# genome-vendor/allpathslg

Hardware: NVIDIA B200
Metric: k-mer spectrum throughput (K=25), k-mer instances counted per second (higher is better)
Workload: dtype u64

## Files before the change

allpathslg_b200/_lib.py:

```python
import ctypes as C
import os

_HERE = os.path.dirname(os.path.abspath(__file__))
LIB_PATH = os.path.join(_HERE, "libapgk.so")

APGK_OK = 0
E_ARG, E_CUDA, E_NOMEM, E_STATE, E_RANGE = -1, -2, -3, -4, -5
WANT_SPECTRUM, WANT_COUNTS, ASYNC_INGEST = 1, 2, 4
N_STAGES = 14
MAX_K = 96


class Config(C.Structure):
    _fields_ = [("K", C.c_int32), ("device", C.c_int32), ("flags", C.c_uint32), ("prefix_bits", C.c_int32),
                ("reserve_bases", C.c_uint64), ("max_round_keys", C.c_uint64),
                ("max_inner_keys", C.c_uint64)]


class GroupStats(C.Structure):
    _fields_ = [("world", C.c_int32), ("n_rounds", C.c_int32), ("n_outer_rounds", C.c_int32), ("prefix_bits", C.c_int32),
                ("split_bits", C.c_int32), ("peer_exchange", C.c_int32), ("shard_instances", C.c_uint64),
                ("remote_bytes", C.c_uint64), ("gather_ms", C.c_float), ("step_ms", C.c_float)]


class GroupFreqStats(C.Structure):
    _fields_ = [("n_batches", C.c_int32), ("n_queries", C.c_uint64), ("remote_bytes", C.c_uint64), ("sweep_ms", C.c_float),
                ("exchange_ms", C.c_float), ("scatter_ms", C.c_float), ("total_ms", C.c_float)]


class SynthParams(C.Structure):
    _fields_ = [("genome_len", C.c_uint64), ("seed_g", C.c_uint64), ("seed_p", C.c_uint64), ("seed_q", C.c_uint64),
                ("seed_r", C.c_uint64), ("seed_e", C.c_uint64), ("read_len", C.c_uint32), ("err_per_200", C.c_uint32)]


_u64p = C.POINTER(C.c_uint64)
_u32p = C.POINTER(C.c_uint32)
_vp = C.c_void_p
SYMBOLS = {
    "apgk_create": (C.c_int, [C.POINTER(Config), C.POINTER(_vp)]),
    "apgk_destroy": (None, [_vp]),
    "apgk_last_error": (C.c_char_p, [_vp]),
    "apgk_words_per_kmer": (C.c_int, [C.c_int]),
    "apgk_reset": (C.c_int, [_vp]),
    "apgk_add_reads": (C.c_int, [_vp, _vp, _vp, C.c_uint64]),
    "apgk_add_reads_uniform": (C.c_int, [_vp, _vp, C.c_uint64, C.c_uint64, C.c_uint32]),
    "apgk_synth_reads": (C.c_int, [_vp, C.POINTER(SynthParams), C.c_uint64, C.c_uint64]),
    "apgk_export_reads": (C.c_int, [_vp, _vp]),
    "apgk_read_store_info": (C.c_int, [_vp, _u64p, _u64p]),
    "apgk_finish": (C.c_int, [_vp]),
    "apgk_totals": (C.c_int, [_vp, _u64p, _u64p]),
    "apgk_spectrum": (C.c_int, [_vp, C.POINTER(_u64p), _u64p]),
    "apgk_spectrum_sparse": (C.c_int, [_vp, C.POINTER(_u64p), C.POINTER(_u64p), _u64p]),
    "apgk_counts_device": (C.c_int, [_vp, C.POINTER(_vp), C.POINTER(_vp), _u64p]),
    "apgk_counts_copy": (C.c_int, [_vp, C.c_uint64, C.c_uint64, _vp, _vp]),
    "apgk_reserve_table": (C.c_int, [_vp, C.c_uint64]),
    "apgk_release_temp": (C.c_int, [_vp]),
    "apgk_prefix_range": (C.c_int, [_vp, C.c_int32, C.c_uint64, _u64p, _u64p]),
    "apgk_lookup": (C.c_int, [_vp, _vp, C.c_uint64, C.c_int, _vp]),
    "apgk_read_freqs": (C.c_int, [_vp, C.c_uint64, C.c_uint64, _vp]),
    "apgk_read_freqs_device": (C.c_int, [_vp, _vp, C.POINTER(C.c_float)]),
    "apgk_build_occurrences": (C.c_int, [_vp]),
    "apgk_occurrences_info": (C.c_int, [_vp, _u64p, _u64p, C.POINTER(C.c_float)]),
    "apgk_occurrences_device": (C.c_int, [_vp, C.POINTER(_vp), C.POINTER(_vp), _u64p]),
    "apgk_occurrences_copy": (C.c_int, [_vp, C.c_uint64, C.c_uint64, _vp, _vp, _vp]),
    "apgk_owner_plan": (C.c_int, [_vp, C.c_uint32, _vp]),
    "apgk_owner_scatter": (C.c_int, [_vp, _vp]),
    "apgk_key_buffer": (C.c_int, [_vp, C.c_uint64, C.POINTER(_vp)]),
    "apgk_owner_of": (C.c_int, [C.c_int, _vp, C.c_uint64, C.c_uint32, _vp]),
    "apgk_finish_keys_device": (C.c_int, [_vp, _vp, C.c_uint64]),
    "apgk_window_upper": (C.c_int, [_vp, C.POINTER(C.c_uint64)]),
    "apgk_choose_prefix_bits": (C.c_int, [_vp, C.c_uint64, C.POINTER(C.c_int32)]),
    "apgk_partition": (C.c_int, [_vp, C.c_int32]),
    "apgk_partition_range": (C.c_int, [_vp, C.c_int32, C.c_int32, C.c_int32]),
    "apgk_level0_totals": (C.c_int, [_vp, _vp, C.c_uint32, C.POINTER(C.c_uint32), C.POINTER(C.c_uint64)]),
    "apgk_partition_info": (C.c_int, [_vp, C.POINTER(_vp), C.POINTER(C.c_uint64), C.POINTER(_vp), C.POINTER(C.c_uint32),
                                      C.POINTER(C.c_uint64)]),
    "apgk_count_pieces": (C.c_int, [_vp, _vp, C.c_uint32, _vp, _vp, C.c_uint64, C.c_uint64, C.c_int32]),
    "apgk_count_pieces_peer": (C.c_int, [_vp, _vp, C.c_uint32, _vp, _vp, C.c_uint64, C.c_uint64, C.c_int32, _vp]),
    "apgk_partition_subsizes": (C.c_int, [_vp, C.c_int32, C.POINTER(C.c_int32), C.POINTER(_vp)]),
    "apgk_partition_export": (C.c_int, [_vp, _vp]),
    "apgk_peer_open": (C.c_int, [_vp, _vp, C.POINTER(_vp)]),
    "apgk_peer_close": (C.c_int, [_vp, _vp]),
    "apgk_group_unique_id": (C.c_int, [_vp]),
    "apgk_group_join": (C.c_int, [_vp, _vp, C.c_int32, C.c_int32, C.POINTER(_vp)]),
    "apgk_group_local": (C.c_int, [C.POINTER(_vp), C.c_int32, C.POINTER(_vp)]),
    "apgk_group_destroy": (None, [_vp]),
    "apgk_group_last_error": (C.c_char_p, [_vp]),
    "apgk_group_count": (C.c_int, [_vp]),
    "apgk_group_totals": (C.c_int, [_vp, _u64p, _u64p]),
    "apgk_group_spectrum_sparse": (C.c_int, [_vp, C.POINTER(_u64p), C.POINTER(_u64p), _u64p]),
    "apgk_group_stats_get": (C.c_int, [_vp, C.POINTER(GroupStats)]),
    "apgk_group_read_freqs_device": (C.c_int, [_vp, _vp, _vp, _vp, C.POINTER(GroupFreqStats)]),
    "apgk_spectrum_device": (C.c_int, [_vp, C.POINTER(_vp), _u64p]),
    "apgk_spectrum_reload": (C.c_int, [_vp]),
    "apgk_stage_ms": (C.c_int, [_vp, C.POINTER(C.c_float)]),
    "apgk_stage_name": (C.c_char_p, [C.c_int]),
    "apgk_kernel_launches": (C.c_uint64, [_vp]),
    "apgk_reset_counters": (None, [_vp]),
    "apgk_geometry": (C.c_int, [_vp, C.POINTER(C.c_int32)]),
    "apgk_device_alloc": (C.c_int, [_vp, C.POINTER(_vp), C.c_size_t]),
    "apgk_device_free": (C.c_int, [_vp, _vp]),
    "apgk_device_copy_to_host": (C.c_int, [_vp, _vp, _vp, C.c_size_t]),
    "apgk_host_alloc": (C.c_int, [C.POINTER(_vp), C.c_size_t]),
    "apgk_host_free": (C.c_int, [_vp]),
    "apgk_debug_counters": (C.c_int, [_vp, _vp, C.c_int]),
    "apgk_debug_host_extract": (C.c_int, [_vp, _vp, C.c_uint64, C.c_int, _vp, _vp]),
    "apgk_debug_host_topdigits": (C.c_int, [_vp, _vp, C.c_uint64, C.c_int, C.c_int, _vp]),
    "apgk_debug_host_canonical": (C.c_int, [C.c_int, _vp, C.c_uint64, _vp]),
    "apgk_debug_host_table_find": (C.c_int, [C.c_int, _vp, C.c_uint64, C.c_int, _vp, C.c_uint64, _vp]),
    "apgk_debug_host_splitters": (C.c_int, [_vp, C.c_uint32, C.c_uint32, C.c_uint32, _vp]),
    "apgk_debug_host_synth": (C.c_int, [C.POINTER(SynthParams), C.c_uint64, C.c_uint64, _vp]),
}

_lib = None


def lib():
    global _lib
    if _lib is None:
        if not os.path.exists(LIB_PATH):
            raise RuntimeError(
                "libapgk.so is missing at %s: build it with `python -c 'import __graft_entry__ as g; g.build()'` "
                "or `make -C allpathslg_b200/csrc`.  There is no CPU fallback." % LIB_PATH)
        L = C.CDLL(LIB_PATH)
        for name, (res, args) in SYMBOLS.items():
            f = getattr(L, name)
            f.restype = res
            f.argtypes = args
        _lib = L
    return _lib
```

allpathslg_b200/csrc/apgk.cu:

```cuda
#include <algorithm>
#include <array>
#include <cmath>
#include <cstdio>
#include <cstdlib>
#include <cstring>
#include <ctime>
#include <map>
#include <string>
#include <type_traits>
#include <utility>
#include <vector>

#include "../../include/apgk.h"
#include "gfreq.cuh"

using namespace apgk;

namespace {

enum Stage { ST_HIST0, ST_SCAN0, ST_SCATTER0, ST_HIST1, ST_SCAN1, ST_SCATTER1, ST_LOCAL, ST_BIG, ST_TABLE, ST_SPECTRUM,
             ST_OWNER, ST_TOTAL, ST_PLAN, ST_REDUCE };
const char* kStageNames[APGK_N_STAGES] = {"hist0", "scan0", "scatter0", "hist1", "scan1", "scatter1",
                                          "local", "big", "table", "spectrum", "owner", "total", "plan", "reduce"};

// ... 114 lines not shown
    char b__[512];                             \
    snprintf(b__, sizeof b__, __VA_ARGS__);    \
    c->err = b__;                              \
    return (code);                             \
  } while (0)

static const bool kSyncDebug = getenv("APGK_SYNC_DEBUG") != nullptr;
#define LAUNCHED() do { c->launches++; CU(cudaGetLastError()); if (kSyncDebug) CU(cudaStreamSynchronize(c->stream)); } while (0)

static const bool kTrace = getenv("APGK_TRACE") != nullptr;
static double trace_now() {
  timespec ts; clock_gettime(CLOCK_MONOTONIC, &ts);
  return ts.tv_sec * 1e3 + ts.tv_nsec * 1e-6;
}
void stages_reset(apgk_ctx* c) {
  c->n_ivs = 0;
  for (int s = 0; s < APGK_N_STAGES; s++) { c->stage_ms[s] = 0; c->open_iv[s] = -1; }
}
void stage_begin(apgk_ctx* c, int s) {
  if (c->n_ivs == c->ivs.size()) {
    apgk_ctx::StageIv iv{s, nullptr, nullptr, false};
    if (cudaEventCreate(&iv.e0) != cudaSuccess || cudaEventCreate(&iv.e1) != cudaSuccess) return;
    c->ivs.push_back(iv);
  }
  apgk_ctx::StageIv& iv = c->ivs[c->n_ivs];
  iv.stage = s; iv.ended = false;
  c->open_iv[s] = (int)c->n_ivs++;
  if (kTrace) fprintf(stderr, "[apgk %.2f] begin %s\n", trace_now(), kStageNames[s]);
  cudaEventRecord(iv.e0, c->stream);
}
void stage_end(apgk_ctx* c, int s) {
  const int i = c->open_iv[s];
  if (i < 0) return;
  cudaEventRecord(c->ivs[i].e1, c->stream);
  c->ivs[i].ended = true;
  c->open_iv[s] = -1;
  if (kTrace) fprintf(stderr, "[apgk %.2f] end   %s\n", trace_now(), kStageNames[s]);
}
void stages_collect(apgk_ctx* c) {
  for (size_t i = 0; i < c->n_ivs; i++) {
    float ms = 0;
    if (c->ivs[i].ended && cudaEventElapsedTime(&ms, c->ivs[i].e0, c->ivs[i].e1) == cudaSuccess) c->stage_ms[c->ivs[i].stage] += ms;
  }
  c->n_ivs = 0;
}

int words_for(int K) { return (2 * K + 63) / 64; }

template <int W> struct Geo;
#ifndef APGK_NT
#define APGK_NT 1024
#endif
template <> struct Geo<1> { static constexpr int NTS = APGK_NT; static constexpr int NPOS = 16; static constexpr int NT0 = APGK_NT; static constexpr int NT1 = APGK_NT; static constexpr uint32_t TILE1 = APGK_NT * 16; static constexpr int LM_KEY = 4096; };
template <> struct Geo<2> { static constexpr int NTS = 1024; static constexpr int NPOS = 8; static constexpr int NT0 = 512; static constexpr int NT1 = 512; static constexpr uint32_t TILE1 = 512 * 8;  static constexpr int LM_KEY = 2048; };
template <> struct Geo<3> { static constexpr int NTS = 1024; static constexpr int NPOS = 4; static constexpr int NT0 = 256; static constexpr int NT1 = 512; static constexpr uint32_t TILE1 = 512 * 5;  static constexpr int LM_KEY = 2048; };
constexpr int LM_U32 = 5120;
constexpr int LM_KEY4 = 3072;
static bool use_local4(int W) {
  static const bool off = getenv("APGK_NO_LOCAL4") != nullptr;
  static const bool all = getenv("APGK_LOCAL4") != nullptr && !strcmp(getenv("APGK_LOCAL4"), "all");
  return !off && (W == 1 || all);
}
constexpr int L3_NT = 512;
constexpr int COL_NT = 1024;

void build_plan(HostPlan& hp, const std::vector<uint64_t>& seg_sizes, uint32_t tile_elems, int bins) {
  const int S = (int)seg_sizes.size();
  hp.seg_tile0.assign(S + 1, 0); hp.seg_chunk0.assign(S + 1, 0); hp.seg_start.assign(S + 1, 0);
  uint64_t max_tiles = 1;
  for (int s = 0; s < S; s++) {
    uint64_t t = (seg_sizes[s] + tile_elems - 1) / tile_elems;
    hp.seg_tile0[s + 1] = hp.seg_tile0[s] + (uint32_t)t;
    hp.seg_start[s + 1] = hp.seg_start[s] + seg_sizes[s];
    max_tiles = std::max(max_tiles, t);
  }
  int ct = (int)((max_tiles + 3) / 4);
  ct = std::max(8, std::min(ct, 128));
  if (const char* e = getenv("APGK_CT")) { if (atoi(e) > 0) ct = atoi(e); }
  for (int s = 0; s < S; s++) {
    uint32_t t = hp.seg_tile0[s + 1] - hp.seg_tile0[s];
    hp.seg_chunk0[s + 1] = hp.seg_chunk0[s] + (t + ct - 1) / ct;
  }
  hp.lp.bins = bins; hp.lp.n_segments = S; hp.lp.chunk_tiles = ct;
  hp.lp.n_tiles = hp.seg_tile0[S]; hp.lp.n_chunks = hp.seg_chunk0[S]; hp.lp.tile_elems = tile_elems;
}

int column_scan(apgk_ctx* c, const HostPlan& hp, int fold, unsigned long long* bofs_out) {
  const LevelPlan& lp = hp.lp;
  if (lp.n_chunks == 0) return APGK_OK;
  CU(c->segtot.ensure((size_t)lp.n_segments * lp.bins * 8));
  CU(c->bstart32.ensure((size_t)lp.n_segments * lp.bins * 4));
  k_segscan<COL_NT><<<lp.n_segments, COL_NT, 0, c->stream>>>(lp, c->chunksum.as<uint32_t>(),
                                                            c->segtot.as<unsigned long long>(),
                                                            c->bstart32.as<uint32_t>(), bofs_out, fold);
  LAUNCHED();
  return APGK_OK;
}

template <typename K>
int set_smem(apgk_ctx* c, K kernel, size_t bytes) {
  if (bytes > 48 * 1024) CU(cudaFuncSetAttribute(kernel, cudaFuncAttributeMaxDynamicSharedMemorySize, (int)bytes));
  return APGK_OK;
}

ReadStore read_store(const apgk_ctx* c) {
  ReadStore rs;
  rs.bases32 = c->bases.as<uint32_t>();
  rs.starts32 = c->starts.as<uint32_t>();
  rs.total_bases = c->total_bases;
  rs.K = c->cfg.K;
  return rs;
}

int wait_ingest(apgk_ctx* c) {
  if (c->n_slices) {
    CU(cudaStreamWaitEvent(c->stream, c->slice_ev[c->n_slices - 1], 0));
    c->n_slices = 0;
  }
  return APGK_OK;
}

int choose_prefix_bits(const apgk_ctx* c, uint64_t upper, int local_max, bool l3) {
  if (c->cfg.prefix_bits > 0) return std::max(2, std::min(24, (int)c->cfg.prefix_bits));
  const char* env = getenv("APGK_PREFIX_BITS");
  if (env && atoi(env) > 0) return std::max(2, std::min(24, atoi(env)));
  double target = l3 ? local_max * 1.0 : local_max / 2.2;
  int P = 2;
  while (P < 24 && (double)upper / (double)(1ull << P) > target) P++;
  return P;
}

void make_geom(apgk_ctx* c, int P) {
  KeyGeom& g = c->geom;
  g.K = c->cfg.K; g.W = c->W;
  g.TB = std::max(2 * g.K, P);
  g.pad = g.TB - 2 * g.K;
  g.D0 = (P + 1) / 2;
  if (const char* e = getenv("APGK_D0")) { if (atoi(e) >= 1 && atoi(e) < P && atoi(e) <= 12 && P - atoi(e) <= 12) g.D0 = atoi(e); }
  g.D1 = P - g.D0;
  g.REM = g.TB - P;
  g.topbits = 2 * g.K - 64 * (g.W - 1);
}

int ensure_store(apgk_ctx* c, uint64_t bases_needed) {
  const size_t bbytes = ((bases_needed + 31) / 32) * 8 + 256;
  const size_t sbytes = ((bases_needed + 31) / 32) * 4 + 256;
  if (bbytes > c->bases.cap) {
    DevBuf nb, ns;
    size_t grow = std::max(bbytes, c->bases.cap * 2);
    CU(cudaStreamSynchronize(c->stream));
    cudaError_t e = nb.ensure(grow, true);
    if (e == cudaSuccess) e = ns.ensure(grow / 2 + 256, true);
    if (e == cudaSuccess && c->total_bases) {
      e = cudaMemcpyAsync(nb.p, c->bases.p, ((c->total_bases + 31) / 32) * 8 + 8, cudaMemcpyDeviceToDevice, c->stream);
      if (e == cudaSuccess) e = cudaMemcpyAsync(ns.p, c->starts.p, ((c->total_bases + 31) / 32) * 4 + 8, cudaMemcpyDeviceToDevice, c->stream);
      if (e == cudaSuccess) e = cudaStreamSynchronize(c->stream);
    }
    if (e != cudaSuccess) { nb.release(); ns.release(); }
    CU(e);
    c->bases.release(); c->starts.release();
    c->bases = nb; c->starts = ns;
  }
  (void)sbytes;
  return APGK_OK;
}

int append_bases(apgk_ctx* c, const uint8_t* packed, uint64_t first_base, uint64_t n_bases) {
  if (!n_bases) return APGK_OK;
  int rc = ensure_store(c, c->total_bases + n_bases);
  if (rc) return rc;
  const uint64_t dst_bit0 = 2 * c->total_bases, src_bit0 = 2 * first_base;
  if ((dst_bit0 & 7) == 0 && (src_bit0 & 7) == 0) {
    const size_t nbytes = (size_t)((2 * n_bases + 7) / 8);
    CU(cudaMemcpyAsync(c->bases.as<uint8_t>() + (dst_bit0 >> 3), packed + (src_bit0 >> 3), nbytes,
                       cudaMemcpyHostToDevice, c->stream));
    if ((2 * n_bases) & 7) {
      uint8_t last = packed[(src_bit0 >> 3) + nbytes - 1] & (uint8_t)((1u << ((2 * n_bases) & 7)) - 1u);
      CU(cudaMemcpyAsync(c->bases.as<uint8_t>() + (dst_bit0 >> 3) + nbytes - 1, &last, 1, cudaMemcpyHostToDevice,
                         c->stream));
      CU(cudaStreamSynchronize(c->stream));
    }
  } else {
    const uint64_t sb_byte = src_bit0 >> 3;
    const uint64_t sb_al = sb_byte & ~7ull;
    const size_t nbytes = (size_t)(((src_bit0 + 2 * n_bases + 7) >> 3) - sb_al);
    CU(c->staging.ensure(nbytes + 32));
    CU(cudaMemsetAsync((uint8_t*)c->staging.p + (nbytes & ~(size_t)7), 0, 24, c->stream));
    CU(cudaMemcpyAsync(c->staging.p, packed + sb_al, nbytes, cudaMemcpyHostToDevice, c->stream));
    const uint64_t nbits = 2 * n_bases;
    const uint64_t nwords = ((dst_bit0 + nbits + 63) >> 6) - (dst_bit0 >> 6);
    k_append_bits<<<(unsigned)((nwords + 255) / 256), 256, 0, c->stream>>>(
        c->staging.as<uint64_t>(), src_bit0 - sb_al * 8, c->bases.as<uint64_t>(), dst_bit0, nbits);
    LAUNCHED();
  }
  return APGK_OK;
}

void invalidate_results(apgk_ctx* c) {
  c->finished = false; c->have_table = false; c->spec_loaded = false;
  c->table_from_reads = false; c->have_occ = false; c->n_occ = 0;
  c->n_instances = c->n_distinct = 0;
  c->owner_ranks = 0;
  c->part_ready = false; c->part_n = 0;
}

enum RunMode { RUN_FULL = 0, RUN_PARTITION = 1 };
template <int W, typename ElemB>
int run_levels(apgk_ctx* c, const Key<W>* dev_keys, uint64_t n_keys, RunMode mode);
template <int W, typename ElemB>
int count_buckets(apgk_ctx* c, uint64_t Nr, uint64_t N_all, uint64_t& n_prev, Key<W>* tmp_keys, bool nosync);

uint64_t window_upper(const apgk_ctx* c) { return c->n_windows; }

template <int W>
bool select_geometry(apgk_ctx* c, uint64_t upper, int forced_P) {
  int lm_u32 = LM_U32;
  if (const char* e = getenv("APGK_LM")) { if (atoi(e) >= 256 && atoi(e) <= 12288) lm_u32 = atoi(e); }
  if (upper == 0) upper = 1;
  if (forced_P > 0) {
    make_geom(c, std::max(2, std::min(24, forced_P)));
    return W == 1 && c->geom.REM <= 32;
  }
  int P = choose_prefix_bits(c, upper, lm_u32, true);
  make_geom(c, P);
  if (W == 1 && c->cfg.prefix_bits <= 0 && !getenv("APGK_PREFIX_BITS")) {
    while (c->geom.REM > 31 && c->geom.REM <= 34 && P < 24) make_geom(c, ++P);
  }
  const bool u32 = (W == 1 && c->geom.REM <= 32);
  if (!u32) {
    P = use_local4(W) ? choose_prefix_bits(c, upper, LM_KEY4 * 3 / 4, true) : choose_prefix_bits(c, upper, Geo<W>::LM_KEY, false);
    make_geom(c, P);
  }
  return u32;
}

template <int W> int compact_table(apgk_ctx* c, uint64_t total);

enum { RES_RANGE_N = 0, RES_SUM_TOT0 = 1, RES_FLAGS = 2, RES_DISTINCT = 3, RES_TABLE_OVF = 4, RES_XFLAGS = 5, RES_WORDS = 16 };

int fetch_results(apgk_ctx* c) {
  CU(cudaMemcpyAsync(c->res_host, c->res.p, RES_WORDS * 8, cudaMemcpyDeviceToHost, c->stream));
  CU(cudaStreamSynchronize(c->stream));
  return APGK_OK;
}

int step_epilogue(apgk_ctx* c, bool full) {
  { int r2 = fetch_results(c); if (r2) return r2; }
  if (c->res_host[RES_FLAGS] & 1ull) FAIL(APGK_E_RANGE, "a level-0 bucket holds 2^32 or more k-mers");
  if (c->res_host[RES_SUM_TOT0] && c->res_host[RES_SUM_TOT0] != c->n_windows_run)
    FAIL(APGK_E_STATE, "internal: level-0 histogram counts %llu k-mers, the input holds %llu",
         (unsigned long long)c->res_host[RES_SUM_TOT0], (unsigned long long)c->n_windows_run);
  if (full && c->table_pending) {
    c->table_pending = false;
    const uint64_t total = c->res_host[RES_DISTINCT];
    if (c->res_host[RES_TABLE_OVF]) {
      int rc = APGK_E_ARG;
      switch (c->W) {
        case 1: rc = compact_table<1>(c, total); break;
        case 2: rc = compact_table<2>(c, total); break;
        case 3: rc = compact_table<3>(c, total); break;
      }
      if (rc) return rc;
      CU(cudaStreamSynchronize(c->stream));
    }
    c->n_distinct = total;
  }
  return APGK_OK;
}

template <int W>
int finish_impl(apgk_ctx* c, const Key<W>* dev_keys, uint64_t n_keys, RunMode mode = RUN_FULL, int forced_P = 0) {
  invalidate_results(c);
  stages_reset(c);
  select_geometry<W>(c, dev_keys ? n_keys : window_upper(c), forced_P);
  if (!c->res_host) CU(cudaHostAlloc((void**)&c->res_host, RES_WORDS * 8, cudaHostAllocDefault));
  CU(c->res.ensure(RES_WORDS * 8));
  CU(cudaMemsetAsync(c->res.p, 0, RES_WORDS * 8, c->stream));
  stage_begin(c, ST_TOTAL);
  int rc;
  if constexpr (W == 1) {
    if (c->geom.REM <= 32) rc = run_levels<W, uint32_t>(c, dev_keys, n_keys, mode);
    else rc = run_levels<W, Key<W>>(c, dev_keys, n_keys, mode);
  } else {
    rc = run_levels<W, Key<W>>(c, dev_keys, n_keys, mode);
  }
  if (rc) {
    if (c->n_slices && c->copy_stream) cudaStreamSynchronize(c->copy_stream);
    c->n_slices = 0;
    cudaStreamSynchronize(c->stream);
    c->n_ivs = 0; c->table_pending = false;
    return rc;
  }
  stage_end(c, ST_TOTAL);
  c->n_deferred = 0;
  if (mode == RUN_FULL && c->deferred.p && c->n_instances)
    CU(cudaMemcpyAsync(&c->n_deferred, c->deferred.p, 4, cudaMemcpyDeviceToHost, c->stream));
  { int r2 = step_epilogue(c, mode == RUN_FULL); if (r2) return r2; }
  stages_collect(c);
  if (mode == RUN_FULL) c->finished = true;
  else c->part_ready = true;
  return APGK_OK;
}

template <typename ElemB, int W>
struct ScatterSel {
  static auto kernel() { return k_scatter_keys<Key<W>, ElemB, Geo<W>::NT1, DIGIT_BITS, false>; }
};

__global__ void k_accumulate_u64(unsigned long long* __restrict__ dst, const unsigned long long* __restrict__ src, uint64_t n) {
  const uint64_t i = (uint64_t)blockIdx.x * blockDim.x + threadIdx.x;
  if (i < n) dst[i] += src[i];
}

int ensure_preserve(apgk_ctx* c, DevBuf& b, size_t bytes, size_t keep_bytes) {
  if (bytes <= b.cap) return APGK_OK;
  if (!keep_bytes || !b.p) { CU(b.ensure(bytes)); return APGK_OK; }
  DevBuf nb;
  if (nb.ensure(std::max(bytes, b.cap + b.cap / 2)) != cudaSuccess) {
    cudaGetLastError();
    CU(nb.ensure(bytes));
  }
  CU(cudaMemcpyAsync(nb.p, b.p, keep_bytes, cudaMemcpyDeviceToDevice, c->stream));
  CU(cudaStreamSynchronize(c->stream));
  b.release();
  b = nb;
  return APGK_OK;
}

template <typename K>
int kernel_setup(apgk_ctx* c, K kernel, int nt, size_t smem, int* occ_out) {
  const auto key = std::make_pair((const void*)kernel, smem);
  auto it = c->kattr.find(key);
  if (it == c->kattr.end()) {
    if (smem > 48 * 1024) CU(cudaFuncSetAttribute(kernel, cudaFuncAttributeMaxDynamicSharedMemorySize, (int)smem));
    int occ = 1;
    CU(cudaOccupancyMaxActiveBlocksPerMultiprocessor(&occ, kernel, nt, smem));
    it = c->kattr.emplace(key, std::max(occ, 1)).first;
  }
  if (occ_out) *occ_out = it->second;
  return APGK_OK;
}

int chunk_tiles_for(uint64_t avg_tiles) {
  int ct = (int)std::min<uint64_t>((2 * avg_tiles + 3) / 4, 128);
  ct = std::max(8, ct);
  if (const char* e = getenv("APGK_CT")) { if (atoi(e) > 0) ct = atoi(e); }
  return ct;
}

template <int W>
int level0_hist(apgk_ctx* c, const Key<W>* dev_keys, uint64_t n_keys, DigitFn<DIGIT_BITS>& dg0) {
  const KeyGeom g = c->geom;
  const int bins0 = 1 << g.D0;
  const uint32_t tile0 = dev_keys ? Geo<W>::TILE1 : (uint32_t)Geo<W>::NT0 * POS_PER_THREAD;
  const uint64_t n_elems = dev_keys ? n_keys : c->total_bases;
  HostPlan& hp0 = c->hp0;
  if (c->hp0_elems != n_elems || c->hp0_tile != tile0 || hp0.lp.bins != bins0 || !c->plan0.p) {
    std::vector<uint64_t> one{n_elems};
    build_plan(hp0, one, tile0, bins0);
    const size_t S1 = hp0.seg_tile0.size();
    CU(c->plan0.ensure(S1 * 16 + 64));
    unsigned char* d = c->plan0.as<unsigned char>();
    CU(cudaMemcpyAsync(d, hp0.seg_start.data(), S1 * 8, cudaMemcpyHostToDevice, c->stream));
    CU(cudaMemcpyAsync(d + S1 * 8, hp0.seg_tile0.data(), S1 * 4, cudaMemcpyHostToDevice, c->stream));
    CU(cudaMemcpyAsync(d + S1 * 12, hp0.seg_chunk0.data(), S1 * 4, cudaMemcpyHostToDevice, c->stream));
    hp0.lp.seg_start = (const uint64_t*)d;
    hp0.lp.seg_tile0 = (const uint32_t*)(d + S1 * 8);
    hp0.lp.seg_chunk0 = (const uint32_t*)(d + S1 * 12);
    c->hp0_elems = n_elems; c->hp0_tile = tile0;
  }
  CU(c->chunksum0.ensure((size_t)hp0.lp.n_chunks * bins0 * 4));
  stage_begin(c, ST_HIST0);
  if (dev_keys) {
    k_hist_keys<Key<W>, Geo<W>::NT1, DIGIT_BITS><<<hp0.lp.n_chunks, Geo<W>::NT1, bins0 * 4, c->stream>>>(
        dev_keys, hp0.lp, dg0, c->chunksum0.as<uint32_t>());
  } else {
    const int top_bits = (g.pad == 0 && g.D0 <= 16 && c->cfg.K >= (g.D0 + 1) / 2 && !getenv("APGK_NO_TOPDIGITS")) ? g.D0 : 0;
    if (c->n_slices == 0) {
      k_hist_reads<W, Geo<W>::NT0, DIGIT_BITS><<<hp0.lp.n_chunks, Geo<W>::NT0, bins0 * 4, c->stream>>>(
          read_store(c), dg0, hp0.lp, top_bits, c->chunksum0.as<uint32_t>());
    } else {
      const uint64_t reach = (uint64_t)c->cfg.K + 256;
      uint32_t c_lo = 0;
      for (size_t i = 0; i < c->n_slices; i++) {
        CU(cudaStreamWaitEvent(c->stream, c->slice_ev[i], 0));
        uint32_t c_hi = hp0.lp.n_chunks;
        if (i + 1 < c->n_slices) {
          const uint64_t safe = c->slice_end[i] > reach ? c->slice_end[i] - reach : 0;
          c_hi = (uint32_t)std::min<uint64_t>(hp0.lp.n_chunks, safe / ((uint64_t)tile0 * hp0.lp.chunk_tiles));
        }
        if (c_hi > c_lo) {
          k_hist_reads<W, Geo<W>::NT0, DIGIT_BITS><<<c_hi - c_lo, Geo<W>::NT0, bins0 * 4, c->stream>>>(
              read_store(c), dg0, hp0.lp, top_bits, c->chunksum0.as<uint32_t>(), c_lo);
          c->launches++;
          c_lo = c_hi;
        }
      }
      c->n_slices = 0;
    }
  }
  LAUNCHED();
  stage_end(c, ST_HIST0);
  stage_begin(c, ST_SCAN0);
  CU(c->tot0_dev.ensure((size_t)bins0 * 8));
  CU(c->bstart32.ensure((size_t)bins0 * 4));
  k_segscan<COL_NT><<<1, COL_NT, 0, c->stream>>>(hp0.lp, c->chunksum0.as<uint32_t>(), c->tot0_dev.as<unsigned long long>(),
                                                 c->bstart32.as<uint32_t>(), nullptr, 0);
  LAUNCHED();
  stage_end(c, ST_SCAN0);
  return APGK_OK;
}

template <int W>
int level0_scatter(apgk_ctx* c, const Key<W>* dev_keys, DigitFn<DIGIT_BITS> dg0, int lo, int hi, uint64_t n_round) {
  const KeyGeom g = c->geom;
  const int bins0 = 1 << g.D0;
  const bool filter = lo > 0 || hi < bins0;
  const HostPlan& hp0 = c->hp0;
  const uint32_t tile0 = hp0.lp.tile_elems;
  CU(c->A.ensure(std::max<size_t>(n_round, 1) * sizeof(Key<W>)));
  CU(c->bstart64.ensure(((size_t)bins0 + 1) * 8));
  stage_begin(c, ST_SCAN0);
  k_plan_range<<<1, PLAN_NT, 0, c->stream>>>(c->tot0_dev.as<unsigned long long>(), bins0, lo, hi, 1u, 1u,
                                            c->bstart64.as<unsigned long long>(), nullptr, nullptr, c->res.as<unsigned long long>());
  LAUNCHED();
  stage_end(c, ST_SCAN0);
  dg0.flo = (uint32_t)lo; dg0.fwidth = (uint32_t)(hi - lo);
  stage_begin(c, ST_SCATTER0);
  const size_t sm = scatter_smem_bytes<Key<W>>(tile0, bins0);
  if (dev_keys) {
    auto launch = [&](auto kern) -> int {
      { int rc = kernel_setup(c, kern, Geo<W>::NT1, sm, nullptr); if (rc) return rc; }
      kern<<<hp0.lp.n_chunks, Geo<W>::NT1, sm, c->stream>>>(dev_keys, hp0.lp, dg0, c->chunksum0.as<uint32_t>(),
                                                            c->bstart64.as<uint64_t>(), 0, 0, c->A.as<Key<W>>());
      return APGK_OK;
    };
    int rc = filter ? launch(k_scatter_keys<Key<W>, Key<W>, Geo<W>::NT1, DIGIT_BITS, true>)
                    : launch(k_scatter_keys<Key<W>, Key<W>, Geo<W>::NT1, DIGIT_BITS, false>);
    if (rc) return rc;
  } else {
    auto launch = [&](auto kern) -> int {
      { int rc = kernel_setup(c, kern, Geo<W>::NTS, sm, nullptr); if (rc) return rc; }
      kern<<<hp0.lp.n_chunks, Geo<W>::NTS, sm, c->stream>>>(read_store(c), dg0, hp0.lp, c->chunksum0.as<uint32_t>(),
                                                            c->bstart64.as<uint64_t>(), c->A.as<Key<W>>());
      return APGK_OK;
    };
    int rc = filter ? launch(k_scatter_reads<W, Geo<W>::NTS, DIGIT_BITS, true, Geo<W>::NPOS>)
                    : launch(k_scatter_reads<W, Geo<W>::NTS, DIGIT_BITS, false, Geo<W>::NPOS>);
    if (rc) return rc;
  }
  LAUNCHED();
  stage_end(c, ST_SCATTER0);
  return APGK_OK;
}

template <int W, typename ElemB>
int level1(apgk_ctx* c, int s_lo, int s_hi, uint64_t n_range, const Key<W>* a_src, int d2) {
  const KeyGeom g = c->geom;
  const int bins0 = 1 << g.D0, bins1 = 1 << g.D1;
  const uint32_t tile = Geo<W>::TILE1;
  const int n_seg_in = std::max(1, s_hi - s_lo);
  const int ct = chunk_tiles_for(n_range / tile / (uint64_t)n_seg_in);
  const uint64_t tiles_bound = n_range / tile + (uint64_t)n_seg_in;
  const uint32_t chunks_bound = (uint32_t)(tiles_bound / (uint64_t)ct + (uint64_t)n_seg_in + 1);
  const size_t S1 = (size_t)bins0 + 1;
  CU(c->plan.ensure(S1 * 16 + 64));
  unsigned char* d = c->plan.as<unsigned char>();
  LevelPlan lp{};
  lp.bins = bins1; lp.n_segments = bins0; lp.chunk_tiles = ct; lp.tile_elems = tile;
  lp.n_tiles = (uint32_t)tiles_bound; lp.n_chunks = chunks_bound;
  lp.seg_start = (const uint64_t*)d;
  lp.seg_tile0 = (const uint32_t*)(d + S1 * 8);
  lp.seg_chunk0 = (const uint32_t*)(d + S1 * 12);
  DigitSpec ds1{DIGIT_BITS, g.TB - g.D0 - g.D1, g.D1, g.pad, 0};
  const DigitFn<DIGIT_BITS> dg1 = make_digit_fn<DIGIT_BITS>(ds1);
  DigitSpec dsw{DIGIT_BITS, g.TB - g.D0 - g.D1 - d2, g.D1 + d2, g.pad, 0};
  const DigitFn<DIGIT_BITS> dgw = make_digit_fn<DIGIT_BITS>(dsw);
  stage_begin(c, ST_SCAN1);
  k_plan_range<<<1, PLAN_NT, 0, c->stream>>>(c->tot0_dev.as<unsigned long long>(), bins0, s_lo, s_hi, tile, (uint32_t)ct,
                                            (unsigned long long*)d, (uint32_t*)(d + S1 * 8), (uint32_t*)(d + S1 * 12), nullptr);
  LAUNCHED();
  stage_end(c, ST_SCAN1);
  CU(c->chunksum.ensure((size_t)chunks_bound * bins1 * 4));
  CU(c->segtot.ensure((size_t)c->nb1 * 8));
  CU(c->bstart32.ensure((size_t)c->nb1 * 4));
  CU(c->bofs.ensure(((size_t)c->nb1 + 1) * 8));
  if (d2 > 0) {
    CU(c->sub_sizes.ensure(((size_t)c->nb1 << d2) * 4 + 16));
    CU(cudaMemsetAsync(c->sub_sizes.p, 0, ((size_t)c->nb1 << d2) * 4, c->stream));
  }
  stage_begin(c, ST_HIST1);
  {
    auto kern = k_hist_keys<Key<W>, Geo<W>::NT1, DIGIT_BITS>;
    const size_t smh = ((size_t)bins1 << d2) * 4;
    { int rc = kernel_setup(c, kern, Geo<W>::NT1, smh, nullptr); if (rc) return rc; }
    kern<<<chunks_bound, Geo<W>::NT1, smh, c->stream>>>(a_src, lp, dg1, c->chunksum.as<uint32_t>(), dgw, d2,
                                                        d2 > 0 ? c->sub_sizes.as<uint32_t>() : nullptr);
    LAUNCHED();
  }
  stage_end(c, ST_HIST1);
  stage_begin(c, ST_SCAN1);
  k_segscan<COL_NT><<<bins0, COL_NT, 0, c->stream>>>(lp, c->chunksum.as<uint32_t>(), c->segtot.as<unsigned long long>(),
                                                     c->bstart32.as<uint32_t>(), c->bofs.as<unsigned long long>(), 1);
  LAUNCHED();
  stage_end(c, ST_SCAN1);
  CU(c->B.ensure(std::max<size_t>(n_range, 1) * sizeof(ElemB) + 16));
  stage_begin(c, ST_SCATTER1);
  {
    const char* eb = getenv("APGK_BULK");
    const bool bulk = eb && !strcmp(eb, "1");
    const size_t smb = scatter_bulk_smem_bytes<ElemB>(tile, bins1);
    if (bulk && sizeof(ElemB) == 4 && smb <= 200 * 1024 && bins1 <= Geo<W>::NT1) {
      auto kern = k_scatter_keys_bulk<Key<W>, ElemB, Geo<W>::NT1, DIGIT_BITS, false>;
      { int rc = kernel_setup(c, kern, Geo<W>::NT1, smb, nullptr); if (rc) return rc; }
      kern<<<chunks_bound, Geo<W>::NT1, smb, c->stream>>>(a_src, lp, dg1, c->chunksum.as<uint32_t>(), nullptr, g.pad, g.REM,
                                                          c->B.as<ElemB>());
    } else {
      auto kern = ScatterSel<ElemB, W>::kernel();
      const size_t sm = scatter_smem_bytes<Key<W>>(tile, bins1);
      { int rc = kernel_setup(c, kern, Geo<W>::NT1, sm, nullptr); if (rc) return rc; }
      kern<<<chunks_bound, Geo<W>::NT1, sm, c->stream>>>(a_src, lp, dg1, c->chunksum.as<uint32_t>(), nullptr, g.pad, g.REM,
                                                         c->B.as<ElemB>());
    }
    LAUNCHED();
  }
  stage_end(c, ST_SCATTER1);
  return APGK_OK;
}

int temp_budget(apgk_ctx* c, size_t* budget) {
  size_t fr = 0, tot = 0;
  CU(cudaMemGetInfo(&fr, &tot));
  const size_t held = c->A.cap + c->B.cap + c->T.cap;
  *budget = (size_t)((double)(fr + held) * 0.60);
  return APGK_OK;
}

template <int W, typename ElemB>
int run_levels(apgk_ctx* c, const Key<W>* dev_keys, uint64_t n_keys, RunMode mode) {
  const KeyGeom g = c->geom;
  const int bins0 = 1 << g.D0, bins1 = 1 << g.D1;
  int local_max = std::is_same<ElemB, uint32_t>::value ? LM_U32 : (use_local4(W) ? LM_KEY4 : Geo<W>::LM_KEY);
  if (std::is_same<ElemB, uint32_t>::value) {
    if (const char* e = getenv("APGK_LM")) { if (atoi(e) >= 256 && atoi(e) <= 12288) local_max = atoi(e); }
  }
  const int want_table = (c->cfg.flags & APGK_WANT_COUNTS) ? 1 : 0;
  c->elem_bytes = sizeof(ElemB);
  c->local_max = (uint32_t)local_max;
  c->nb1 = (uint32_t)bins0 * (uint32_t)bins1;
  c->n_rounds = 0; c->n_big = 0; c->n_distinct = 0;
  c->table_pending = false;
  CU(c->spec_dense.ensure((size_t)SPEC_DENSE * 8));
  CU(cudaMemsetAsync(c->spec_dense.p, 0, (size_t)SPEC_DENSE * 8, c->stream));
  CU(c->out_off.ensure(((size_t)c->nb1 + 1) * 8));
  CU(cudaMemsetAsync(c->out_off.p, 0, ((size_t)c->nb1 + 1) * 8, c->stream));
  const uint64_t N = dev_keys ? n_keys : c->n_windows;
  c->n_instances = N; c->n_windows_run = N;
  c->tot0_host.assign((size_t)bins0, 0);
  if (N == 0) {
    { int rc = wait_ingest(c); if (rc) return rc; }
    c->have_table = want_table != 0;
    c->part_n = 0;
    if (mode == RUN_PARTITION) {
      CU(c->segtot.ensure((size_t)c->nb1 * 8));
      CU(cudaMemsetAsync(c->segtot.p, 0, (size_t)c->nb1 * 8, c->stream));
    }
    return APGK_OK;
  }

  DigitSpec ds0{DIGIT_BITS, g.TB - g.D0, g.D0, g.pad, 0};
  DigitFn<DIGIT_BITS> dg0 = make_digit_fn<DIGIT_BITS>(ds0);
  { int rc = level0_hist<W>(c, dev_keys, n_keys, dg0); if (rc) return rc; }

  const size_t eA = sizeof(Key<W>), eB = sizeof(ElemB) + (want_table ? 4 : 0);
  uint64_t cap_outer = c->cfg.max_round_keys, cap_inner = c->cfg.max_inner_keys;
  if (const char* e = getenv("APGK_ROUND_KEYS")) { if (atoll(e) > 0) cap_outer = (uint64_t)atoll(e); }
  if (const char* e = getenv("APGK_INNER_KEYS")) { if (atoll(e) > 0) cap_inner = (uint64_t)atoll(e); }
  bool single;
  if (cap_outer) {
    if (!cap_inner) cap_inner = cap_outer;
    single = N <= cap_outer && N <= cap_inner;
    c->last_cap_keys = std::min(cap_outer, cap_inner);
  } else {
    single = N * (eA + eB) <= c->A.cap + c->B.cap + c->T.cap && N * eA <= c->A.cap && N * sizeof(ElemB) <= c->B.cap;
    if (!single || mode == RUN_PARTITION) {
      size_t budget = 0;
      { int rc = temp_budget(c, &budget); if (rc) return rc; }
      c->last_cap_keys = (uint64_t)(budget / (eA + eB));
      single = N <= c->last_cap_keys;
      if (!single) {
        const uint64_t ci = cap_inner;
        cap_outer = ci ? (budget > ci * eB ? (budget - ci * eB) / eA : 1) : (uint64_t)((double)budget / ((double)eA + (double)eB / 4.0));
        cap_inner = ci ? ci : std::max<uint64_t>(1, cap_outer / 4);
        cap_outer = std::max<uint64_t>(cap_outer, 1);
      }
    }
  }
  const bool forced_range = mode == RUN_PARTITION && c->force_d0_lo >= 0;
  struct Round { int lo, hi; uint64_t n; std::vector<std::array<uint64_t, 3>> inner; };
  std::vector<Round> rounds;
  std::vector<uint64_t>& tot0 = c->tot0_host;
  if (!single || mode == RUN_PARTITION) {
    CU(cudaMemcpyAsync(tot0.data(), c->tot0_dev.p, (size_t)bins0 * 8, cudaMemcpyDeviceToHost, c->stream));
    CU(cudaStreamSynchronize(c->stream));
    uint64_t sum = 0;
    for (int d = 0; d < bins0; d++) {
      if (tot0[d] >= (1ull << 32)) FAIL(APGK_E_RANGE, "level-0 bucket %d holds %llu k-mers (>= 2^32)", d, (unsigned long long)tot0[d]);
      sum += tot0[d];
    }
    if (sum != N) FAIL(APGK_E_STATE, "internal: level-0 histogram counts %llu k-mers, expected %llu", (unsigned long long)sum, (unsigned long long)N);
  }
  if (forced_range) {
    Round r;
    r.lo = std::min(c->force_d0_lo, bins0); r.hi = std::min(std::max(c->force_d0_hi, c->force_d0_lo), bins0);
    r.n = 0;
    for (int d = r.lo; d < r.hi; d++) r.n += tot0[d];
    r.inner.push_back({(uint64_t)r.lo, (uint64_t)r.hi, r.n});
    rounds.push_back(r);
  } else if (single) {
    Round r{0, bins0, N, {}};
    r.inner.push_back({0, (uint64_t)bins0, N});
    rounds.push_back(r);
  } else {
    int lo = 0; uint64_t acc = 0;
    auto close_outer = [&](int hi) {
      Round r{lo, hi, acc, {}};
      int ilo = lo; uint64_t iacc = 0;
      for (int d = lo; d < hi; d++) {
        if (iacc && iacc + tot0[d] > cap_inner) { r.inner.push_back({(uint64_t)ilo, (uint64_t)d, iacc}); ilo = d; iacc = 0; }
        iacc += tot0[d];
      }
      r.inner.push_back({(uint64_t)ilo, (uint64_t)hi, iacc});
      rounds.push_back(r);
    };
    for (int d = 0; d < bins0; d++) {
      if (acc && acc + tot0[d] > cap_outer) { close_outer(d); lo = d; acc = 0; }
      acc += tot0[d];
    }
    close_outer(bins0);
  }
  for (const Round& r : rounds) c->n_rounds += (uint32_t)r.inner.size();
  if (mode == RUN_PARTITION && !forced_range && !single)
    FAIL(APGK_E_RANGE, "apgk_partition: %u k-mer-space rounds would be needed; the sharded exchange takes one", c->n_rounds);

  CU(c->spec_ovf.ensure(((size_t)N / SPEC_DENSE + 16) * 8));
  CU(cudaMemsetAsync(c->spec_ovf.p, 0, 8, c->stream));
  CU(c->nd.ensure(((size_t)c->nb1 + 1) * 4));
  CU(c->out_off_local.ensure(((size_t)c->nb1 + 1) * 8));
  CU(c->stats.ensure(64));
  uint64_t n_prev = 0;
  uint64_t n_counted = 0;

  for (const Round& r : rounds) {
    if (r.n == 0) {
      if (mode == RUN_PARTITION) {
        CU(c->segtot.ensure((size_t)c->nb1 * 8));
        CU(cudaMemsetAsync(c->segtot.p, 0, (size_t)c->nb1 * 8, c->stream));
        c->part_n = 0;
        return APGK_OK;
      }
      continue;
    }
    { int rc = level0_scatter<W>(c, dev_keys, dg0, r.lo, r.hi, r.n); if (rc) return rc; }
    uint64_t off_a = 0;
    for (const auto& in : r.inner) {
      n_counted += in[2];
      const uint64_t n_in = in[2];
      if (n_in == 0) continue;
      Key<W>* a_src = c->A.as<Key<W>>() + off_a;
      { int rc = level1<W, ElemB>(c, (int)in[0], (int)in[1], n_in, a_src, 0); if (rc) return rc; }
      if (mode == RUN_PARTITION) { c->part_n = n_in; return APGK_OK; }
      c->count_src = c->B.p; c->bucket_lo = c->bucket_hi = 0;
      if (!single) { c->bucket_lo = (uint32_t)in[0] * (uint32_t)bins1; c->bucket_hi = (uint32_t)in[1] * (uint32_t)bins1; }
      c->table_scale = single ? 1.0 : std::max(1.0, (double)N / (double)std::max<uint64_t>(n_counted, 1));
      { int rc = count_buckets<W, ElemB>(c, n_in, N, n_prev, a_src, single); if (rc) return rc; }
      c->table_scale = 1.0;
      c->bucket_lo = c->bucket_hi = 0;
      off_a += n_in;
    }
  }
  if (!single) c->n_distinct = n_prev;
  c->have_table = want_table != 0;
  return APGK_OK;
}

template <int W>
int compact_table(apgk_ctx* c, uint64_t total) {
  CU(c->out_keys.ensure(std::max<size_t>(total + (total >> 5), 1) * sizeof(Key<W>)));
  CU(c->out_cnt.ensure(std::max<size_t>(total + (total >> 5), 1) * 4));
  k_compact<W><<<c->n_sm * 8, 256, 0, c->stream>>>(c->tmp_keys_last ? (const Key<W>*)c->tmp_keys_last : c->A.as<Key<W>>(), c->T.as<uint32_t>(),
                                                   c->bofs.as<unsigned long long>(), c->out_off_local.as<unsigned long long>(), c->nb1,
                                                   c->out_keys.as<Key<W>>(), c->out_cnt.as<uint32_t>(), nullptr, 0ull, nullptr);
  LAUNCHED();
  return APGK_OK;
}

template <int W, typename ElemB>
int count_buckets(apgk_ctx* c, uint64_t Nr, uint64_t N, uint64_t& n_prev, Key<W>* tmp_keys, bool nosync) {
  const KeyGeom g = c->geom;
  const int local_max = (int)c->local_max;
  int l3_nt = L3_NT;
  if (std::is_same<ElemB, uint32_t>::value) {
    if (const char* e = getenv("APGK_L3_NT")) { if (atoi(e) == 256 || atoi(e) == 512) l3_nt = atoi(e); }
  }
  const bool use_l3 = std::is_same<ElemB, uint32_t>::value && g.REM >= 1 && g.REM <= 31;
  const bool use_l4 = !std::is_same<ElemB, uint32_t>::value && use_local4(W) && g.pad == 0 && g.REM >= 1;
  const int want_table = (c->cfg.flags & APGK_WANT_COUNTS) ? 1 : 0;
  const uint32_t big_cap = (uint32_t)(Nr / local_max + 16);
  uint64_t n_big = 0;
  unsigned long long stats[2] = {0, 0};
  if (!(use_l3 || use_l4)) {
    CU(c->big_list.ensure((size_t)big_cap * 4));
    CU(cudaMemsetAsync(c->stats.p, 0, 64, c->stream));
    k_classify<<<(c->nb1 + 255) / 256, 256, 0, c->stream>>>(c->segtot.as<unsigned long long>(), c->nb1, (uint32_t)local_max,
                                                           c->big_list.as<uint32_t>(), big_cap, c->stats.as<unsigned long long>());
    LAUNCHED();
    CU(cudaMemcpyAsync(stats, c->stats.p, 16, cudaMemcpyDeviceToHost, c->stream));
    CU(cudaStreamSynchronize(c->stream));
    n_big = stats[0];
    c->n_big += n_big;
  }
  {
    EmitCtx<W> ec;
    ec.want_table = want_table; ec.rem_bits = g.REM; ec.pad = g.pad;
    ec.tmp_keys = tmp_keys;
    c->tmp_keys_last = tmp_keys;
    if (want_table) CU(c->T.ensure(std::max<size_t>(Nr, 1) * 4));
    ec.tmp_cnt = c->T.as<uint32_t>();
    ec.spec_dense = c->spec_dense.as<unsigned long long>();
    ec.spec_ovf = c->spec_ovf.as<unsigned long long>();
    ec.spec_ovf_cap = (uint32_t)(N / SPEC_DENSE + 8);
    BucketTable bt;
    bt.bofs = c->bofs.as<unsigned long long>();
    bt.bsize = c->segtot.as<unsigned long long>();
    bt.nb = c->bucket_hi ? c->bucket_hi : c->nb1; bt.local_max = (uint32_t)local_max; bt.b0 = c->bucket_hi ? c->bucket_lo : 0;
    if (c->bucket_hi) CU(cudaMemsetAsync(c->nd.p, 0, ((size_t)c->nb1 + 1) * 4, c->stream));
    CU(c->deferred.ensure(((size_t)c->nb1 + 1) * 4));
    CU(cudaMemsetAsync(c->deferred.p, 0, 4, c->stream));
    stage_begin(c, ST_LOCAL);
    if (use_l3) {
      if constexpr (std::is_same<ElemB, uint32_t>::value) {
        auto launch3 = [&](auto kern3, int nt) -> int {
          const size_t sm3 = Local3Smem::bytes(local_max);
          int occ3 = 1;
          { int rc = kernel_setup(c, kern3, nt, sm3, &occ3); if (rc) return rc; }
          const uint32_t grid3 = std::min<uint32_t>(c->nb1, (uint32_t)(c->n_sm * std::max(occ3, 1)));
          kern3<<<grid3, nt, sm3, c->stream>>>((const uint32_t*)c->count_src, bt, g.REM, ec, c->nd.as<uint32_t>());
          return APGK_OK;
        };
        int rc3 = l3_nt == 256 ? launch3(k_local3<256, W>, 256) : launch3(k_local3<512, W>, 512);
        if (rc3) return rc3;
        LAUNCHED();
      }
    } else if (use_l4) {
      if constexpr (!std::is_same<ElemB, uint32_t>::value) {
        auto kern4 = k_local4<512, W>;
        const size_t sm4 = Local4Smem::bytes(local_max, W);
        int occ4 = 1;
        { int rc = kernel_setup(c, kern4, 512, sm4, &occ4); if (rc) return rc; }
        const uint32_t grid4 = std::min<uint32_t>(c->nb1, (uint32_t)(c->n_sm * std::max(occ4, 1)));
        kern4<<<grid4, 512, sm4, c->stream>>>((const Key<W>*)c->count_src, bt, g.REM, ec, c->nd.as<uint32_t>());
        LAUNCHED();
      }
    } else {
      auto kern2 = k_local2<ElemB, W>;
      const size_t sm2 = Local2Smem<ElemB>::bytes(local_max);
      int occ2 = 1;
      { int rc = kernel_setup(c, kern2, L2_NT, sm2, &occ2); if (rc) return rc; }
      const uint32_t grid2 = std::min<uint32_t>(c->nb1, (uint32_t)(c->n_sm * std::max(occ2, 1)));
      kern2<<<grid2, L2_NT, sm2, c->stream>>>((const ElemB*)c->count_src, bt, g.REM, ec, c->nd.as<uint32_t>(),
                                              c->deferred.as<uint32_t>(), c->nb1);
      LAUNCHED();
      auto kern = k_local<ElemB, W>;
      const size_t sm = LocalSmem<ElemB>::bytes(local_max);
      int occ = 1;
      { int rc = kernel_setup(c, kern, LOCAL_NT, sm, &occ); if (rc) return rc; }
      const uint32_t grid = std::min<uint32_t>(c->nb1, (uint32_t)(c->n_sm * std::max(occ, 1)));
      kern<<<grid, LOCAL_NT, sm, c->stream>>>((const ElemB*)c->count_src, bt, g.REM, ec, c->nd.as<uint32_t>(),
                                              c->deferred.as<uint32_t>(), c->nb1);
      LAUNCHED();
    }
    stage_end(c, ST_LOCAL);
    if (n_big) {
      if (n_big > big_cap) FAIL(APGK_E_RANGE, "internal: oversize bucket list overflow");
      auto kern = k_big<ElemB, W>;
      const size_t sm = LocalSmem<ElemB>::bytes(local_max);
      int occ = 1;
      { int rc = kernel_setup(c, kern, LOCAL_NT, sm, &occ); if (rc) return rc; }
      const uint32_t grid = (uint32_t)std::min<uint64_t>(n_big, (uint64_t)c->n_sm * std::max(occ, 1));
      CU(c->scratch.ensure((size_t)stats[1] * sizeof(ElemB) + 16));
      CU(c->stacks.ensure((size_t)grid * BIG_STACK * 16));
      CU(c->misc.ensure(64));
      CU(cudaMemsetAsync(c->misc.p, 0, 64, c->stream));
      BigParams bp;
      bp.big_list = c->big_list.as<uint32_t>();
      bp.n_big = (const uint32_t*)c->stats.p;
      bp.ticket = c->misc.as<unsigned int>();
      bp.scratch_cursor = (unsigned long long*)(c->misc.as<unsigned char>() + 8);
      bp.scratch = c->scratch.p;
      bp.stacks = c->stacks.as<unsigned long long>();
      stage_begin(c, ST_BIG);
      kern<<<grid, LOCAL_NT, sm, c->stream>>>((ElemB*)c->count_src, bt, g.REM, ec, c->nd.as<uint32_t>(), bp);
      LAUNCHED();
      stage_end(c, ST_BIG);
    }

    stage_begin(c, ST_TABLE);
    {
      const uint64_t n = c->nb1;
      const uint32_t nblocks = (uint32_t)((n + 1 + SCAN_BLOCK - 1) / SCAN_BLOCK);
      CU(c->blocksum.ensure(((size_t)nblocks + 1) * 8));
      unsigned long long* res = c->res.as<unsigned long long>();
      k_scan_blocksum<<<nblocks, SCAN_NT, 0, c->stream>>>(c->nd.as<uint32_t>(), n, c->blocksum.as<unsigned long long>());
      LAUNCHED();
      k_scan_top<<<1, SCAN_NT, 0, c->stream>>>(c->blocksum.as<unsigned long long>(), nblocks, res ? res + RES_DISTINCT : nullptr);
      LAUNCHED();
      k_scan_apply<<<nblocks, SCAN_NT, 0, c->stream>>>(c->nd.as<uint32_t>(), n, c->blocksum.as<unsigned long long>(),
                                                       c->out_off_local.as<unsigned long long>());
      LAUNCHED();
      k_accumulate_u64<<<(unsigned)((n + 1 + 255) / 256), 256, 0, c->stream>>>(c->out_off.as<unsigned long long>(),
                                                                              c->out_off_local.as<unsigned long long>(), n + 1);
      LAUNCHED();
      const bool optimistic = nosync && n_prev == 0 && (!want_table || (c->out_keys.cap && c->out_cnt.cap));
      if (optimistic) {
        if (want_table) {
          const unsigned long long cap = std::min<unsigned long long>(c->out_keys.cap / sizeof(Key<W>), c->out_cnt.cap / 4);
// ... 1083 lines not shown
  if (d_run_off) *d_run_off = c->occ_off.as<uint64_t>();
  if (d_occ) *d_occ = c->n_occ ? c->occ.as<uint64_t>() : nullptr;
  if (n_occ) *n_occ = c->n_occ;
  return APGK_OK;
}

int apgk_occurrences_copy(apgk_ctx* c, uint64_t first_kmer, uint64_t n_kmers, uint64_t* run_off_out, uint32_t* read_id_out,
                          int32_t* pos_out) {
  if (!c) return APGK_E_ARG;
  if (!c->have_occ) FAIL(APGK_E_STATE, "no occurrences: call apgk_build_occurrences first");
  if (first_kmer > c->n_distinct || n_kmers > c->n_distinct - first_kmer) FAIL(APGK_E_ARG, "k-mer range beyond the table");
  CU(cudaSetDevice(c->device));
  return occurrences_copy_impl(c, first_kmer, n_kmers, run_off_out, read_id_out, pos_out);
}

int apgk_read_freqs_device(apgk_ctx* c, uint32_t* d_out, float* ms3) {
  if (!c || !d_out) return APGK_E_ARG;
  if (!c->finished || !c->have_table) FAIL(APGK_E_STATE, "no table: finish with APGK_WANT_COUNTS first");
  if (!c->table_from_reads)
    FAIL(APGK_E_STATE, "the bulk form needs a table counted from this context's read store (apgk_finish, not a shard or a key array)");
  CU(cudaSetDevice(c->device));
  for (float& m : c->freq_ms) m = 0;
  int rc;
  if (kFreqDirect) {
    { int r2 = wait_ingest(c); if (r2) return r2; }
    for (cudaEvent_t& e : c->occ_ev) if (!e) CU(cudaEventCreate(&e));
    CU(cudaEventRecord(c->occ_ev[0], c->stream));
    constexpr int NT = 128;
    const uint64_t threads = (c->total_bases + POS_PER_THREAD - 1) / POS_PER_THREAD;
    if (threads) {
      switch (c->W) {
        case 1: k_read_freqs<1, NT><<<(unsigned)((threads + NT - 1) / NT), NT, 0, c->stream>>>(read_store(c), freq_table<1>(c), 0, c->total_bases, d_out); break;
        case 2: k_read_freqs<2, NT><<<(unsigned)((threads + NT - 1) / NT), NT, 0, c->stream>>>(read_store(c), freq_table<2>(c), 0, c->total_bases, d_out); break;
        case 3: k_read_freqs<3, NT><<<(unsigned)((threads + NT - 1) / NT), NT, 0, c->stream>>>(read_store(c), freq_table<3>(c), 0, c->total_bases, d_out); break;
      }
      LAUNCHED();
    }
    CU(cudaEventRecord(c->occ_ev[1], c->stream));
    CU(cudaStreamSynchronize(c->stream));
    cudaEventElapsedTime(&c->freq_ms[1], c->occ_ev[0], c->occ_ev[1]);
    rc = APGK_OK;
  } else {
    rc = read_freqs_bulk_dispatch(c, d_out);
  }
  if (ms3) for (int i = 0; i < 3; i++) ms3[i] = c->freq_ms[i];
  return rc;
}

int apgk_owner_plan(apgk_ctx* c, uint32_t n_ranks, uint64_t* counts_out) {
  if (!c || !counts_out || n_ranks < 1 || n_ranks > 1024) return APGK_E_ARG;
  CU(cudaSetDevice(c->device));
  switch (c->W) {
    case 1: return owner_plan_impl<1>(c, n_ranks, counts_out);
    case 2: return owner_plan_impl<2>(c, n_ranks, counts_out);
    case 3: return owner_plan_impl<3>(c, n_ranks, counts_out);
  }
  return APGK_E_ARG;
}

int apgk_owner_scatter(apgk_ctx* c, uint64_t* d_keys_out) {
  if (!c) return APGK_E_ARG;
  if (!c->owner_ranks) FAIL(APGK_E_STATE, "apgk_owner_plan has not run");
  CU(cudaSetDevice(c->device));
  switch (c->W) {
    case 1: return owner_scatter_impl<1>(c, d_keys_out);
    case 2: return owner_scatter_impl<2>(c, d_keys_out);
    case 3: return owner_scatter_impl<3>(c, d_keys_out);
  }
  return APGK_E_ARG;
}

int apgk_key_buffer(apgk_ctx* c, uint64_t n_keys, uint64_t** d_ptr) {
  if (!c || !d_ptr) return APGK_E_ARG;
  CU(cudaSetDevice(c->device));
  CU(cudaStreamSynchronize(c->stream));
  CU(c->A.ensure(std::max<size_t>(n_keys, 1) * (size_t)c->W * 8));
  *d_ptr = c->A.as<uint64_t>();
  return APGK_OK;
}

int apgk_owner_of(int K, const uint64_t* kmers, uint64_t n, uint32_t n_ranks, uint32_t* owner_out) {
  if (K < 1 || K > APGK_MAX_K || !kmers || !owner_out || !n_ranks) return APGK_E_ARG;
  const int W = words_for(K);
  for (uint64_t i = 0; i < n; i++) {
    if (W == 1) { Key<1> k; k.w[0] = kmers[i]; owner_out[i] = key_owner(k, n_ranks); }
    else if (W == 2) { Key<2> k; k.w[0] = kmers[2 * i]; k.w[1] = kmers[2 * i + 1]; owner_out[i] = key_owner(k, n_ranks); }
    else { Key<3> k; k.w[0] = kmers[3 * i]; k.w[1] = kmers[3 * i + 1]; k.w[2] = kmers[3 * i + 2]; owner_out[i] = key_owner(k, n_ranks); }
  }
  return APGK_OK;
}

int apgk_spectrum_device(apgk_ctx* c, uint64_t** d_spec, uint64_t* len) {
  if (!c || !d_spec) return APGK_E_ARG;
  if (!c->finished) FAIL(APGK_E_STATE, "apgk_finish has not run");
  *d_spec = c->spec_dense.as<uint64_t>();
  if (len) *len = SPEC_DENSE;
  return APGK_OK;
}

int apgk_spectrum_reload(apgk_ctx* c) {
  if (!c) return APGK_E_ARG;
  c->spec_loaded = false;
  c->spec_host.clear();
  return APGK_OK;
}

int apgk_stage_ms(const apgk_ctx* c, float* ms_out) {
  if (!c || !ms_out) return APGK_E_ARG;
  for (int s = 0; s < APGK_N_STAGES; s++) ms_out[s] = c->stage_ms[s];
  return APGK_OK;
}
const char* apgk_stage_name(int i) { return (i >= 0 && i < APGK_N_STAGES) ? kStageNames[i] : ""; }
uint64_t apgk_kernel_launches(const apgk_ctx* c) { return c ? c->launches : 0; }
void apgk_reset_counters(apgk_ctx* c) { if (c) c->launches = 0; }

int apgk_geometry(const apgk_ctx* c, int32_t* out8) {
  if (!c || !out8) return APGK_E_ARG;
  out8[0] = c->geom.D0; out8[1] = c->geom.D1; out8[2] = c->geom.REM; out8[3] = (int32_t)c->elem_bytes;
  out8[4] = (int32_t)std::min<uint64_t>(c->n_big, 0x7fffffff);
  out8[5] = (int32_t)std::min<uint32_t>(c->n_deferred, 0x7fffffff);
  out8[6] = (int32_t)c->local_max;
  out8[7] = (int32_t)c->n_rounds;
  return APGK_OK;
}

int apgk_device_alloc(apgk_ctx* c, void** p, size_t bytes) {
  if (!c || !p) return APGK_E_ARG;
  CU(cudaSetDevice(c->device));
  CU(cudaMalloc(p, bytes ? bytes : 1));
  return APGK_OK;
}
int apgk_device_free(apgk_ctx* c, void* p) {
  if (!c) return APGK_E_ARG;
  CU(cudaSetDevice(c->device));
  CU(cudaFree(p));
  return APGK_OK;
}
int apgk_device_copy_to_host(apgk_ctx* c, void* dst_host, const void* src_dev, size_t bytes) {
  if (!c || (!dst_host && bytes)) return APGK_E_ARG;
  CU(cudaSetDevice(c->device));
  if (bytes) {
    CU(cudaMemcpyAsync(dst_host, src_dev, bytes, cudaMemcpyDeviceToHost, c->stream));
    CU(cudaStreamSynchronize(c->stream));
  }
  return APGK_OK;
}

int apgk_host_alloc(void** p, size_t bytes) {
  if (!p) return APGK_E_ARG;
  return cudaHostAlloc(p, bytes, cudaHostAllocDefault) == cudaSuccess ? APGK_OK : APGK_E_NOMEM;
}
int apgk_host_free(void* p) { return cudaFreeHost(p) == cudaSuccess ? APGK_OK : APGK_E_CUDA; }


int apgk_group_unique_id(uint8_t id_out[APGK_GROUP_ID_BYTES]) {
  if (!id_out) return APGK_E_ARG;
  static_assert(sizeof(ncclUniqueId) == APGK_GROUP_ID_BYTES, "unique id size");
  if (!g_nccl.load().empty()) return APGK_E_CUDA;
  ncclUniqueId id;
  if (g_nccl.GetUniqueId(&id) != ncclSuccess) return APGK_E_CUDA;
  memcpy(id_out, &id, APGK_GROUP_ID_BYTES);
  return APGK_OK;
}

static int group_init_rank(apgk_group* g, RankState& r, apgk_ctx* c) {
  if (c->group) GFAIL(APGK_E_STATE, "the context already belongs to a group");
  r.c = c;
  c->group = g;
  GCU(cudaSetDevice(c->device));
  GCU(cudaEventCreateWithFlags(&r.ev_a, cudaEventDisableTiming));
  GCU(cudaEventCreateWithFlags(&r.ev_b, cudaEventDisableTiming));
  return APGK_OK;
}

int apgk_group_join(apgk_ctx* ctx, const uint8_t id[APGK_GROUP_ID_BYTES], int32_t rank, int32_t world, apgk_group** out) {
  if (!ctx || !id || !out || world < 1 || world > 1024 || rank < 0 || rank >= world) return APGK_E_ARG;
  *out = nullptr;
  apgk_ctx* c = ctx;
  const std::string e = g_nccl.load();
  if (!e.empty()) FAIL(APGK_E_CUDA, "%s", e.c_str());
  apgk_group* g = new apgk_group();
  g->world = world; g->n_local = 1; g->rank0 = rank; g->use_nccl = true;
  g->rs.resize(1);
  int rc = group_init_rank(g, g->rs[0], ctx);
  if (rc == APGK_OK) {
    ncclUniqueId nid;
    memcpy(&nid, id, APGK_GROUP_ID_BYTES);
    const ncclResult_t r = g_nccl.CommInitRank(&g->comm, world, nid, rank);
    if (r != ncclSuccess) { g->err = std::string("ncclCommInitRank failed: ") + g_nccl.GetErrorString(r); rc = APGK_E_CUDA; }
  }
  if (rc) { c->err = g->err; apgk_group_destroy(g); return rc; }
  *out = g;
  return APGK_OK;
}

int apgk_group_local(apgk_ctx* const* ctxs, int32_t n, apgk_group** out) {
  if (!ctxs || !out || n < 1 || n > 1024) return APGK_E_ARG;
  *out = nullptr;
  for (int i = 0; i < n; i++) if (!ctxs[i]) return APGK_E_ARG;
  apgk_group* g = new apgk_group();
  g->world = n; g->n_local = n; g->rank0 = 0; g->use_nccl = false;
  g->rs.resize(n);
  int rc = APGK_OK;
  for (int i = 0; i < n && rc == APGK_OK; i++) rc = group_init_rank(g, g->rs[i], ctxs[i]);
  for (int i = 0; i < n && rc == APGK_OK; i++)
    for (int j = 0; j < n; j++) {
      const int di = ctxs[i]->device, dj = ctxs[j]->device;
      if (di == dj) continue;
      int can = 0;
      cudaDeviceCanAccessPeer(&can, di, dj);
      if (!can) { g->err = "devices of a single-process group must be peer-accessible"; rc = APGK_E_CUDA; break; }
      cudaSetDevice(di);
      const cudaError_t e = cudaDeviceEnablePeerAccess(dj, 0);
      if (e != cudaSuccess && e != cudaErrorPeerAccessAlreadyEnabled) { g->err = cudaGetErrorString(e); rc = APGK_E_CUDA; break; }
      cudaGetLastError();
    }
  if (rc) { ctxs[0]->err = g->err; apgk_group_destroy(g); return rc; }
  *out = g;
  return APGK_OK;
}

void apgk_group_destroy(apgk_group* g) {
  if (!g) return;
  for (size_t i = 0; i < g->rs.size(); i++)
    if (g->rs[i].c) group_detach(g, g->rs[i].c);
  if (g->comm) g_nccl.CommDestroy(g->comm);
  delete g;
}

const char* apgk_group_last_error(const apgk_group* g) { return g ? g->err.c_str() : "null group"; }

int apgk_group_count(apgk_group* g) {
  if (!g) return APGK_E_ARG;
  return group_count(g);
}

int apgk_group_read_freqs_device(apgk_group* g, uint32_t* const* d_out, const uint64_t* first_base, const uint64_t* n_bases,
                                 apgk_group_freq_stats* stats) {
  if (!g) return APGK_E_ARG;
  return group_read_freqs(g, d_out, first_base, n_bases, stats);
}

int apgk_group_totals(const apgk_group* g, uint64_t* n_instances, uint64_t* n_distinct) {
  if (!g) return APGK_E_ARG;
  if (!g->counted) return APGK_E_STATE;
  if (n_instances) *n_instances = g->n_instances;
  if (n_distinct) *n_distinct = g->n_distinct;
  return APGK_OK;
}

int apgk_group_spectrum_sparse(apgk_group* g, const uint64_t** freq, const uint64_t** n_kmers, uint64_t* n) {
  if (!g) return APGK_E_ARG;
  if (!g->counted) GFAIL(APGK_E_STATE, "apgk_group_count has not run");
  if (freq) *freq = g->sparse_f.data();
  if (n_kmers) *n_kmers = g->sparse_n.data();
  if (n) *n = g->sparse_f.size();
  return APGK_OK;
}

int apgk_group_stats_get(const apgk_group* g, apgk_group_stats* out) {
  if (!g || !out) return APGK_E_ARG;
  if (!g->counted) return APGK_E_STATE;
  *out = g->stats;
  return APGK_OK;
}

int apgk_debug_counters(apgk_ctx* c, uint64_t* out8, int reset) {
  if (!c || !out8) return APGK_E_ARG;
  CU(cudaSetDevice(c->device));
  CU(cudaStreamSynchronize(c->stream));
  CU(cudaMemcpyFromSymbol(out8, g_l4_dbg, 64));
  if (reset) { unsigned long long z[8] = {0}; CU(cudaMemcpyToSymbol(g_l4_dbg, z, 64)); }
  return APGK_OK;
}

int apgk_debug_host_extract(const uint8_t* packed, const uint64_t* off, uint64_t n_reads, int K, uint64_t* kmers_out,
                            uint8_t* valid_out) {
  if (!packed || !off || K < 1 || K > APGK_MAX_K) return APGK_E_ARG;
  if (!n_reads) return APGK_OK;
  switch (words_for(K)) {
    case 1: host_extract<1>(packed, off, n_reads, K, kmers_out, valid_out); break;
    case 2: host_extract<2>(packed, off, n_reads, K, kmers_out, valid_out); break;
    case 3: host_extract<3>(packed, off, n_reads, K, kmers_out, valid_out); break;
  }
  return APGK_OK;
}

int apgk_debug_host_topdigits(const uint8_t* packed, const uint64_t* off, uint64_t n_reads, int K, int D,
                              uint32_t* digits_out) {
  if (!packed || !off || !digits_out || K < 1 || K > APGK_MAX_K || D < 1 || D > 16 || K < (D + 1) / 2 || 2 * K < D)
    return APGK_E_ARG;
  if (!n_reads) return APGK_OK;
  const uint64_t b0 = off[0], total = off[n_reads] - b0;
  std::vector<uint32_t> bases((total + 15) / 16 + 16, 0);
  for (uint64_t q = 0; q < total; q++) {
    const uint64_t s = b0 + q;
    bases[q >> 4] |= (uint32_t)((packed[s >> 2] >> ((s & 3) * 2)) & 3u) << ((q & 15) * 2);
  }
  for (uint64_t p = 0; p < total; p += 16)
    top_digits16(bases.data(), p, K, D, [&](int j, uint32_t d) { if (p + j < total) digits_out[p + j] = d; });
  return APGK_OK;
}

int apgk_debug_host_canonical(int K, const uint64_t* kmers, uint64_t n, uint64_t* out) {
  if (K < 1 || K > APGK_MAX_K) return APGK_E_ARG;
  const int W = words_for(K);
  for (uint64_t i = 0; i < n; i++) {
    if (W == 1) { Key<1> k; k.w[0] = kmers[i]; k = key_canonical(k, K); out[i] = k.w[0]; }
    else if (W == 2) { Key<2> k; memcpy(k.w, kmers + 2 * i, 16); k = key_canonical(k, K); memcpy(out + 2 * i, k.w, 16); }
    else { Key<3> k; memcpy(k.w, kmers + 3 * i, 24); k = key_canonical(k, K); memcpy(out + 3 * i, k.w, 24); }
  }
  return APGK_OK;
}

int apgk_debug_host_table_find(int K, const uint64_t* sorted_kmers, uint64_t n, int prefix_bits, const uint64_t* queries,
                               uint64_t n_q, uint64_t* idx_out) {
  if (K < 1 || K > APGK_MAX_K || prefix_bits < 1 || prefix_bits > 24) return APGK_E_ARG;
  if (words_for(K) > 1 && prefix_bits > 2 * K) return APGK_E_ARG;
  switch (words_for(K)) {
    case 1: host_table_find<1>(K, sorted_kmers, n, prefix_bits, queries, n_q, idx_out); break;
    case 2: host_table_find<2>(K, sorted_kmers, n, prefix_bits, queries, n_q, idx_out); break;
    case 3: host_table_find<3>(K, sorted_kmers, n, prefix_bits, queries, n_q, idx_out); break;
  }
  return APGK_OK;
}

int apgk_debug_host_splitters(const uint32_t* bucket_sizes, uint32_t n_buckets, uint32_t world, uint32_t bucket_cost, uint32_t* bounds_out) {
  if (!bucket_sizes || !bounds_out || !world) return APGK_E_ARG;
  std::vector<unsigned long long> S((size_t)n_buckets + 1, 0);
  for (uint32_t b = 0; b < n_buckets; b++) S[b + 1] = S[b] + (bucket_sizes[b] ? (unsigned long long)bucket_sizes[b] + bucket_cost : 0ull);
  for (uint32_t r = 0; r <= world; r++) bounds_out[r] = splitter_bound(S.data(), n_buckets, world, r);
  return APGK_OK;
}

int apgk_debug_host_synth(const apgk_synth_params* p, uint64_t r0, uint64_t n_reads, uint8_t* packed_out) {
  if (!p || !packed_out) return APGK_E_ARG;
  SynthParams sp{p->genome_len, p->seed_g, p->seed_p, p->seed_q, p->seed_r, p->seed_e, p->read_len, p->err_per_200};
  const uint64_t nb = n_reads * (uint64_t)p->read_len;
  uint32_t* w = (uint32_t*)packed_out;
  for (uint64_t wi = 0; wi * 16 < nb; wi++) w[wi] = synth_word(sp, r0, wi * 16, nb);
  return APGK_OK;
}

}
```

allpathslg_b200/csrc/extract.cuh:

```cuda
#pragma once
#include "kmer_types.cuh"

namespace apgk {

constexpr int POS_PER_THREAD = 16;

template <int W>
struct Window16 {
  uint32_t w[2 * W + 1];
  uint32_t v0;
};

template <int W>
APGK_HD void load_window16(const uint32_t* __restrict__ bases32, uint64_t p, int K, Window16<W>& win) {
  const uint64_t wi = p >> 4;
  const int nw = (K + 15 + 15) >> 4;
#pragma unroll
  for (int m = 0; m < 2 * W + 1; m++) win.w[m] = (m < nw) ? bases32[wi + m] : 0u;
  const uint64_t vi = wi + (uint64_t)(K >> 4);
  const uint32_t ks = 2u * (uint32_t)(K & 15);
  win.v0 = funnel_r(bases32[vi], bases32[vi + 1], ks);
}

template <int W>
APGK_HD void load_window_at(const uint32_t* __restrict__ bases32, uint64_t p, int K, Window16<W>& win) {
  const uint64_t wi = p >> 4;
  const uint32_t sh = 2u * (uint32_t)(p & 15);
  uint32_t raw[2 * W + 2];
#pragma unroll
  for (int m = 0; m < 2 * W + 2; m++) raw[m] = bases32[wi + m];
#pragma unroll
  for (int m = 0; m < 2 * W + 1; m++) win.w[m] = funnel_r(raw[m], raw[m + 1], sh);
  const uint64_t q = p + (uint64_t)K;
  const uint64_t vi = q >> 4;
  const uint32_t ks = 2u * (uint32_t)(q & 15);
  win.v0 = funnel_r(bases32[vi], bases32[vi + 1], ks);
}

template <int W, int NPOS, typename F>
APGK_HD void extractN(const Window16<W>& win, int K, F&& f) {
  const int topbits = 2 * K - 64 * (W - 1);
  const uint64_t topmask = lowmask64(topbits);
  Key<W> fw;
  {
    uint64_t rm[W];
#pragma unroll
    for (int i = 0; i < W; i++) {
      uint64_t x = (uint64_t)win.w[2 * i] | ((uint64_t)win.w[2 * i + 1] << 32);
      rm[i] = swap_pairs(brev64(x));
    }
    const int s = 64 * W - 2 * K;
#pragma unroll
    for (int i = 0; i < W; i++) {
      uint64_t v = rm[i] >> s;
      if (i > 0 && s > 0) v |= rm[i - 1] << (64 - s);
      fw.w[i] = v;
    }
  }
#pragma unroll
  for (int j = 0; j < NPOS; j++) {
    Key<W> rc;
#pragma unroll
    for (int q = 0; q < W; q++) {
      uint32_t lo = funnel_r(win.w[2 * q], win.w[2 * q + 1], 2 * j);
      uint32_t hi = funnel_r(win.w[2 * q + 1], win.w[2 * q + 2], 2 * j);
      rc.w[W - 1 - q] = ~((uint64_t)lo | ((uint64_t)hi << 32));
    }
    rc.w[0] &= topmask;
    const bool use_rc = key_less(rc, fw);
    Key<W> c;
#pragma unroll
    for (int i = 0; i < W; i++) c.w[i] = use_rc ? rc.w[i] : fw.w[i];
    f(j, c, use_rc);
    if (j + 1 < NPOS) {
      const uint64_t b = (win.v0 >> (2 * j)) & 3u;
#pragma unroll
      for (int i = 0; i < W - 1; i++) fw.w[i] = (fw.w[i] << 2) | (fw.w[i + 1] >> 62);
      fw.w[W - 1] = (fw.w[W - 1] << 2) | b;
      fw.w[0] &= topmask;
    }
  }
}

template <int W, typename F>
APGK_HD void extract16(const Window16<W>& win, int K, F&& f) { extractN<W, POS_PER_THREAD>(win, K, static_cast<F&&>(f)); }

template <typename F>
APGK_HD void top_digits16(const uint32_t* __restrict__ bases32, uint64_t p, int K, int D, F&& f) {
  const int nb = (D + 1) >> 1;
  const uint32_t mask = lowmask32(2 * nb);
  const uint64_t wi = p >> 4;
  const uint32_t f0 = bases32[wi], f1 = bases32[wi + 1];
  const uint64_t wf = ((uint64_t)f0 | ((uint64_t)f1 << 32)) >> (2 * nb);
  uint32_t x = f0 & mask;
  x = (uint32_t)(swap_pairs(brev64((uint64_t)x)) >> (64 - 2 * nb));
  const uint64_t q = p + (uint64_t)(K - nb);
  const uint64_t ri = q >> 4;
  const uint32_t rs = 2u * (uint32_t)(q & 15);
  const uint32_t r0 = bases32[ri], r1 = bases32[ri + 1], r2 = bases32[ri + 2];
  const uint32_t u0 = funnel_r(r0, r1, rs), u1 = funnel_r(r1, r2, rs);
  const int drop = 2 * nb - D;
#pragma unroll
  for (int j = 0; j < POS_PER_THREAD; j++) {
    const uint32_t rc_top = ~funnel_r(u0, u1, 2 * j) & mask;
    const uint32_t d = (x < rc_top ? x : rc_top) >> drop;
    f(j, d);
    if (j + 1 < POS_PER_THREAD) x = ((x << 2) | ((uint32_t)(wf >> (2 * j)) & 3u)) & mask;
  }
}

APGK_HD uint32_t window_valid_mask16(const uint32_t* __restrict__ starts32, uint64_t p, int K, uint64_t total_bases) {
  if (p + (uint64_t)K > total_bases) return 0u;
  uint32_t ok = 0xFFFFu;
  const uint64_t room = total_bases - (uint64_t)K - p;
  if (room < 15) ok = (2u << (uint32_t)room) - 1u;
  if (K < 2) return ok;
  const uint64_t lo = p + 1, hi = p + (uint64_t)K + 14;
  uint32_t inv = 0;
  for (uint64_t wi = lo >> 5; wi <= (hi >> 5); wi++) {
    uint32_t bits = starts32[wi];
    if (wi == (lo >> 5)) bits &= 0xFFFFFFFFu << (uint32_t)(lo & 31);
    if (wi == (hi >> 5)) bits &= 0xFFFFFFFFu >> (31u - (uint32_t)(hi & 31));
    while (bits) {
#ifdef __CUDA_ARCH__
      const int b = __ffs((int)bits) - 1;
#else
      const int b = __builtin_ctz(bits);
#endif
      bits &= bits - 1;
      const int s = (int)((wi << 5) + (uint64_t)b - p);
      const int j0 = s - K + 1 > 0 ? s - K + 1 : 0;
      const int j1 = s - 1 < 15 ? s - 1 : 15;
      if (j0 <= j1) inv |= ((2u << j1) - 1u) & ~((1u << j0) - 1u);
    }
  }
  return ok & ~inv;
}

}
```

allpathslg_b200/csrc/partition.cuh:

```cuda
#pragma once
#include "extract.cuh"
#include <cstdio>

#ifdef APGK_CHECKS
#define APGK_CHECK(cond, ...) do { if (!(cond)) { printf(__VA_ARGS__); } } while (0)
#define APGK_OK_OR_SKIP(cond) (cond)
#else
#define APGK_CHECK(cond, ...) do { } while (0)
#define APGK_OK_OR_SKIP(cond) true
#endif

namespace apgk {

__device__ __forceinline__ uint32_t smem_u32(const void* p) { return (uint32_t)__cvta_generic_to_shared(p); }
__device__ __forceinline__ uint32_t atoms_add(uint32_t addr, uint32_t v) {
  uint32_t r;
  asm volatile("atom.shared.add.u32 %0, [%1], %2;" : "=r"(r) : "r"(addr), "r"(v) : "memory");
  return r;
}
__device__ __forceinline__ void reds_add(uint32_t addr, uint32_t v) {
  asm volatile("red.shared.add.u32 [%0], %1;" ::"r"(addr), "r"(v) : "memory");
}
__device__ __forceinline__ uint32_t lds_u32(uint32_t addr) {
  uint32_t r;
  asm volatile("ld.shared.u32 %0, [%1];" : "=r"(r) : "r"(addr) : "memory");
  return r;
}
__device__ __forceinline__ uint64_t lds_u64(uint32_t addr) {
  uint64_t r;
  asm volatile("ld.shared.u64 %0, [%1];" : "=l"(r) : "r"(addr) : "memory");
  return r;
}
__device__ __forceinline__ void sts_u64(uint32_t addr, uint64_t v) {
  asm volatile("st.shared.u64 [%0], %1;" ::"r"(addr), "l"(v) : "memory");
}
template <int W>
__device__ __forceinline__ void sts_key(uint32_t addr, const Key<W>& k) {
#pragma unroll
  for (int i = 0; i < W; i++) sts_u64(addr + 8 * i, k.w[i]);
}
template <int W>
__device__ __forceinline__ Key<W> lds_key(uint32_t addr) {
  Key<W> k;
#pragma unroll
  for (int i = 0; i < W; i++) k.w[i] = lds_u64(addr + 8 * i);
  return k;
}

__device__ __forceinline__ uint32_t atoms_add_if(uint32_t addr, uint32_t v, uint32_t pred) {
  uint32_t r;
  asm volatile("{\n\t.reg .pred p;\n\tsetp.ne.u32 p, %3, 0;\n\tmov.u32 %0, 0;\n\t@p atom.shared.add.u32 %0, [%1], %2;\n\t}"
               : "=r"(r) : "r"(addr), "r"(v), "r"(pred) : "memory");
  return r;
}
__device__ __forceinline__ void sts_u64_if(uint32_t addr, uint64_t v, uint32_t pred) {
  asm volatile("{\n\t.reg .pred p;\n\tsetp.ne.u32 p, %2, 0;\n\t@p st.shared.u64 [%0], %1;\n\t}" ::"r"(addr), "l"(v), "r"(pred) : "memory");
}
__device__ __forceinline__ void sts_u32_if(uint32_t addr, uint32_t v, uint32_t pred) {
  asm volatile("{\n\t.reg .pred p;\n\tsetp.ne.u32 p, %2, 0;\n\t@p st.shared.u32 [%0], %1;\n\t}" ::"r"(addr), "r"(v), "r"(pred) : "memory");
}
__device__ __forceinline__ void stg_u64_if(void* ptr, uint64_t v, uint32_t pred) {
  asm volatile("{\n\t.reg .pred p;\n\tsetp.ne.u32 p, %2, 0;\n\t@p st.global.u64 [%0], %1;\n\t}" ::"l"(ptr), "l"(v), "r"(pred) : "memory");
}
__device__ __forceinline__ void stg_u32_if(void* ptr, uint32_t v, uint32_t pred) {
  asm volatile("{\n\t.reg .pred p;\n\tsetp.ne.u32 p, %2, 0;\n\t@p st.global.u32 [%0], %1;\n\t}" ::"l"(ptr), "r"(v), "r"(pred) : "memory");
}
#ifndef APGK_LD_HINT
#define APGK_LD_HINT 1
#endif
#ifndef APGK_SK_EARLY
#define APGK_SK_EARLY 1
#endif
#ifndef APGK_ST_HINT
#define APGK_ST_HINT 0
#endif
__device__ __forceinline__ uint64_t l2_policy_evict_first() {
  uint64_t p; asm volatile("createpolicy.fractional.L2::evict_first.b64 %0, 1.0;" : "=l"(p)); return p;
}
__device__ __forceinline__ uint64_t l2_policy_evict_last() {
  uint64_t p; asm volatile("createpolicy.fractional.L2::evict_last.b64 %0, 1.0;" : "=l"(p)); return p;
}
__device__ __forceinline__ uint64_t ldg_u64_pol(const void* ptr, uint64_t pol) {
  uint64_t r;
  asm volatile("ld.global.L2::cache_hint.u64 %0, [%1], %2;" : "=l"(r) : "l"(ptr), "l"(pol) : "memory");
  return r;
}
__device__ __forceinline__ void stg_u64_if_pol(void* ptr, uint64_t v, uint32_t pred, uint64_t pol) {
  asm volatile("{\n\t.reg .pred p;\n\tsetp.ne.u32 p, %2, 0;\n\t@p st.global.L2::cache_hint.u64 [%0], %1, %3;\n\t}" ::"l"(ptr), "l"(v), "r"(pred), "l"(pol) : "memory");
}
__device__ __forceinline__ void stg_u32_if_pol(void* ptr, uint32_t v, uint32_t pred, uint64_t pol) {
  asm volatile("{\n\t.reg .pred p;\n\tsetp.ne.u32 p, %2, 0;\n\t@p st.global.L2::cache_hint.u32 [%0], %1, %3;\n\t}" ::"l"(ptr), "r"(v), "r"(pred), "l"(pol) : "memory");
}
template <int W>
__device__ __forceinline__ void stg_if(Key<W>* ptr, const Key<W>& k, uint32_t pred, uint64_t pol) {
#pragma unroll
  for (int i = 0; i < W; i++) {
    if (APGK_ST_HINT) stg_u64_if_pol(&ptr->w[i], k.w[i], pred, pol);
    else stg_u64_if(&ptr->w[i], k.w[i], pred);
  }
}
__device__ __forceinline__ void stg_if(uint32_t* ptr, const uint32_t& k, uint32_t pred, uint64_t pol) {
  if (APGK_ST_HINT) stg_u32_if_pol(ptr, k, pred, pol);
  else stg_u32_if(ptr, k, pred);
}
__device__ __forceinline__ uint32_t ldg_stream(const uint32_t* ptr, uint64_t) { return *ptr; }
template <int W>
__device__ __forceinline__ Key<W> ldg_stream(const Key<W>* ptr, uint64_t pol) {
  if constexpr (APGK_LD_HINT == 0) return *ptr;
  else {
    Key<W> k;
#pragma unroll
    for (int i = 0; i < W; i++) k.w[i] = ldg_u64_pol(&ptr->w[i], pol);
    return k;
  }
}

__device__ __forceinline__ void reds_add_if(uint32_t addr, uint32_t v, uint32_t pred) {
  asm volatile("{\n\t.reg .pred p;\n\tsetp.ne.u32 p, %2, 0;\n\t@p red.shared.add.u32 [%0], %1;\n\t}" ::"r"(addr), "r"(v), "r"(pred) : "memory");
}
__device__ __forceinline__ uint32_t atoms_cas(uint32_t addr, uint32_t cmp, uint32_t val) {
  uint32_t r;
  asm volatile("atom.shared.cas.b32 %0, [%1], %2, %3;" : "=r"(r) : "r"(addr), "r"(cmp), "r"(val) : "memory");
  return r;
}
__device__ __forceinline__ uint32_t atoms_cas_if(uint32_t addr, uint32_t cmp, uint32_t val, uint32_t pred) {
  uint32_t r;
  asm volatile("{\n\t.reg .pred p;\n\tsetp.ne.u32 p, %4, 0;\n\tmov.u32 %0, %3;\n\t@p atom.shared.cas.b32 %0, [%1], %2, %3;\n\t}"
               : "=r"(r) : "r"(addr), "r"(cmp), "r"(val), "r"(pred) : "memory");
  return r;
}

template <typename T> struct SmemElem;
template <int W> struct SmemElem<Key<W>> {
  __device__ __forceinline__ static void st(uint32_t a, const Key<W>& k) { sts_key<W>(a, k); }
  __device__ __forceinline__ static void st_if(uint32_t a, const Key<W>& k, uint32_t pred) {
#pragma unroll
    for (int i = 0; i < W; i++) sts_u64_if(a + 8 * i, k.w[i], pred);
  }
  __device__ __forceinline__ static Key<W> ld(uint32_t a) { return lds_key<W>(a); }
};
template <> struct SmemElem<uint32_t> {
  __device__ __forceinline__ static void st(uint32_t a, const uint32_t& k) {
    asm volatile("st.shared.u32 [%0], %1;" ::"r"(a), "r"(k) : "memory");
  }
  __device__ __forceinline__ static void st_if(uint32_t a, const uint32_t& k, uint32_t pred) { sts_u32_if(a, k, pred); }
  __device__ __forceinline__ static uint32_t ld(uint32_t a) { return lds_u32(a); }
};

constexpr int DIGIT_BITS = 0;
constexpr int DIGIT_OWNER = 1;

struct DigitSpec {
  int mode;
  int pos, len, pad;
  uint32_t n_ranks;
};

template <int MODE>
struct DigitFn {
  int kind;
  int sh;
  uint32_t mask;
  int rsh;
  int pos, len;
  uint32_t n_ranks;
  uint32_t flo, fwidth;
  template <int W>
  __device__ __forceinline__ uint32_t operator()(const Key<W>& k) const {
    if constexpr (MODE == DIGIT_OWNER) return key_owner(k, n_ranks);
    else if constexpr (W == 1) {
      const uint32_t t = (uint32_t)(k.w[0] >> (sh & 63));
      return (t << (kind & 31)) & mask;
    } else return key_bits(k, pos, len);
  }
  __device__ __forceinline__ uint32_t operator()(uint32_t e) const { return (e >> rsh) & mask; }
};
template <int MODE>
inline DigitFn<MODE> make_digit_fn(const DigitSpec& ds) {
  DigitFn<MODE> f;
  const int eff = ds.pos - ds.pad;
  if (eff >= 0) { f.kind = 0; f.sh = eff; }
  else { f.kind = -eff; f.sh = 0; }
  f.mask = lowmask32(ds.len);
  f.rsh = ds.pos;
  f.pos = ds.pos; f.len = ds.len; f.n_ranks = ds.n_ranks;
  f.flo = 0; f.fwidth = 0xFFFFFFFFu;
  return f;
}

template <int NT>
__device__ __forceinline__ uint32_t block_excl_scan(uint32_t v, uint32_t* warp_scratch) {
  const int lane = threadIdx.x & 31, wid = threadIdx.x >> 5;
  uint32_t incl = v;
#pragma unroll
  for (int o = 1; o < 32; o <<= 1) {
    uint32_t u = __shfl_up_sync(0xffffffffu, incl, o);
    if (lane >= o) incl += u;
  }
  __syncthreads();
  if (lane == 31) warp_scratch[wid] = incl;
  __syncthreads();
  if (wid == 0) {
    uint32_t t = lane < NT / 32 ? warp_scratch[lane] : 0u, it = t;
#pragma unroll
    for (int o = 1; o < 32; o <<= 1) {
      uint32_t u = __shfl_up_sync(0xffffffffu, it, o);
      if (lane >= o) it += u;
    }
    warp_scratch[lane] = it - t;
    if (lane == 31) warp_scratch[32] = it;
  }
  __syncthreads();
  return incl - v + warp_scratch[wid];
}

template <int NT>
__device__ __forceinline__ uint32_t block_excl_scan1(uint32_t v, uint32_t* warp_scratch, uint32_t& total_out) {
  const int lane = threadIdx.x & 31, wid = threadIdx.x >> 5;
  uint32_t incl = v;
#pragma unroll
  for (int o = 1; o < 32; o <<= 1) {
    uint32_t u = __shfl_up_sync(0xffffffffu, incl, o);
    if (lane >= o) incl += u;
  }
  if (lane == 31) warp_scratch[wid] = incl;
  __syncthreads();
  uint32_t t = lane < NT / 32 ? warp_scratch[lane] : 0u, it = t;
#pragma unroll
  for (int o = 1; o < 32; o <<= 1) {
    uint32_t u = __shfl_up_sync(0xffffffffu, it, o);
    if (lane >= o) it += u;
  }
  total_out = __shfl_sync(0xffffffffu, it, 31);
  const uint32_t wbase = __shfl_sync(0xffffffffu, it - t, wid);
  return incl - v + wbase;
}

struct LevelPlan {
  int bins;
  int n_segments;
  int chunk_tiles;
  uint32_t n_tiles, n_chunks;
  uint32_t tile_elems;
  const uint32_t* seg_tile0;
  const uint32_t* seg_chunk0;
  const uint64_t* seg_start;
};

__device__ __forceinline__ int seg_of(const uint32_t* __restrict__ arr, int n, uint32_t x) {
  int lo = 0, hi = n;
  while (hi - lo > 1) {
    int mid = (lo + hi) >> 1;
    if (arr[mid] <= x) lo = mid; else hi = mid;
  }
  return lo;
}

__device__ __forceinline__ void chunk_tiles(const LevelPlan& lp, uint32_t c, int& s, uint32_t& t0, uint32_t& t1) {
  s = seg_of(lp.seg_chunk0, lp.n_segments, c);
  t0 = lp.seg_tile0[s] + (c - lp.seg_chunk0[s]) * (uint32_t)lp.chunk_tiles;
  t1 = t0 + (uint32_t)lp.chunk_tiles;
  if (t1 > lp.seg_tile0[s + 1]) t1 = lp.seg_tile0[s + 1];
}

__device__ __forceinline__ void prefetch_l1(const void* p) { asm volatile("prefetch.global.L1 [%0];" ::"l"(p)); }
__device__ __forceinline__ void prefetch_l2(const void* p) { asm volatile("prefetch.global.L2 [%0];" ::"l"(p)); }

struct ReadStore {
  const uint32_t* bases32;
  const uint32_t* starts32;
  uint64_t total_bases;
  int K;
};

template <int W, int NT, int MODE>
__global__ void __launch_bounds__(NT) k_hist_reads(ReadStore rs, DigitFn<MODE> dg, LevelPlan lp, int top_bits,
                                                   uint32_t* __restrict__ chunksum, uint32_t chunk0 = 0) {
  extern __shared__ __align__(16) unsigned char smem_raw[];
  uint32_t* hist = (uint32_t*)smem_raw;
  const int bins = lp.bins;
  for (int i = threadIdx.x; i < bins; i += NT) hist[i] = 0;
  __syncthreads();
  int s; uint32_t t0, t1;
  const uint32_t chunk = blockIdx.x + chunk0;
  chunk_tiles(lp, chunk, s, t0, t1);
  const uint32_t hist_a = smem_u32(hist);
  for (uint32_t t = t0; t < t1; t++) {
    const uint64_t p = ((uint64_t)t * NT + threadIdx.x) * POS_PER_THREAD;
    if (p < rs.total_bases) {
      const uint32_t valid = window_valid_mask16(rs.starts32, p, rs.K, rs.total_bases);
      if (valid) {
        if (MODE == DIGIT_BITS && top_bits > 0) {
          top_digits16(rs.bases32, p, rs.K, top_bits, [&](int j, uint32_t d) {
            if ((valid >> j) & 1u) reds_add(hist_a + 4 * d, 1u);
          });
        } else {
          Window16<W> win;
          load_window16<W>(rs.bases32, p, rs.K, win);
          extract16<W>(win, rs.K, [&](int j, const Key<W>& c, bool) {
            if ((valid >> j) & 1u) reds_add(hist_a + 4 * dg(c), 1u);
          });
        }
      }
    }
  }
  __syncthreads();
  uint32_t* row = chunksum + (size_t)chunk * bins;
  for (int i = threadIdx.x; i < bins; i += NT) row[i] = hist[i];
}

template <typename Elem>
__device__ __forceinline__ void scatter_smem_carve(unsigned char* raw, uint32_t tile_elems, int bins, Elem*& stage,
                                                   uint32_t*& cnt, unsigned long long*& G, unsigned long long*& Gabs,
                                                   uint32_t*& scratch) {
  stage = (Elem*)raw;
  size_t off = ((size_t)tile_elems * sizeof(Elem) + 15) & ~(size_t)15;
  G = (unsigned long long*)(raw + off);
  off += (size_t)bins * 8;
  Gabs = (unsigned long long*)(raw + off);
  off += (size_t)bins * 8;
  cnt = (uint32_t*)(raw + off);
  off += (size_t)bins * 8;
  scratch = (uint32_t*)(raw + off);
}
template <typename Elem>
inline size_t scatter_smem_bytes(uint32_t tile_elems, int bins) {
  return (((size_t)tile_elems * sizeof(Elem) + 15) & ~(size_t)15) + (size_t)bins * 24 + 40 * 4;
}

template <int NT>
__device__ __forceinline__ void chunk_begin(const uint32_t* __restrict__ chunk_row, const uint64_t* __restrict__ bstart64,
                                            uint64_t seg_base, int bins, unsigned long long* Gabs, uint32_t* cnt) {
  const int per = (bins + NT - 1) / NT;
  for (int j = 0; j < per; j++) {
    const int d = threadIdx.x * per + j;
    if (d < bins) {
      unsigned long long g = seg_base + chunk_row[d];
      if (bstart64) g += bstart64[d];
      Gabs[d] = g;
      cnt[d] = 0;
      cnt[bins + d] = 0;
    }
  }
}
template <int NT>
__device__ __forceinline__ uint32_t tile_scan(int bins, unsigned long long* G, unsigned long long* Gabs, uint32_t* cur,
                                              uint32_t* nxt, uint32_t* scratch) {
  const int per = (bins + NT - 1) / NT;
  const int d0 = threadIdx.x * per;
  uint32_t sum = 0;
  for (int j = 0; j < per; j++) {
    const int d = d0 + j;
    if (d < bins) sum += cur[d];
  }
  uint32_t total;
  uint32_t excl = block_excl_scan1<NT>(sum, scratch, total);
  for (int j = 0; j < per; j++) {
    const int d = d0 + j;
    if (d < bins) {
      const uint32_t c = cur[d];
      const unsigned long long ga = Gabs[d];
      cur[d] = excl;
      G[d] = ga - excl;
      Gabs[d] = ga + c;
      nxt[d] = 0;
      excl += c;
    }
  }
  __syncthreads();
  return total;
}

template <int W, int NT, int MODE, bool FILTER, int NPOS = POS_PER_THREAD>
__global__ void __launch_bounds__(NT, (NT <= 512 ? 2 : 1)) k_scatter_reads(ReadStore rs, DigitFn<MODE> dg, LevelPlan lp,
                                                      const uint32_t* __restrict__ chunkpref,
                                                      const uint64_t* __restrict__ bstart64, Key<W>* __restrict__ out) {
  extern __shared__ __align__(16) unsigned char smem_raw[];
  Key<W>* stage; uint32_t* cnt2; unsigned long long* G; unsigned long long* Gabs; uint32_t* scratch;
  const int bins = lp.bins;
  scatter_smem_carve<Key<W>>(smem_raw, NT * NPOS, bins, stage, cnt2, G, Gabs, scratch);
  int s; uint32_t t0, t1;
  chunk_tiles(lp, blockIdx.x, s, t0, t1);
  chunk_begin<NT>(chunkpref + (size_t)blockIdx.x * bins, bstart64, 0ull, bins, Gabs, cnt2);
  constexpr uint32_t ES = (uint32_t)sizeof(Key<W>);
  const uint32_t stage_a = smem_u32(stage), G_a = smem_u32(G), cnt2_a = smem_u32(cnt2);
  const uint64_t pol_st = APGK_ST_HINT == 1 ? l2_policy_evict_last() : (APGK_ST_HINT == 2 ? l2_policy_evict_first() : 0ull);
  Key<W> key[NPOS];
  uint32_t rk[NPOS / 2];
  uint32_t valid = 0;
  auto extract_rank = [&](uint32_t t, uint32_t cnt_a, auto&& between) {
    const uint64_t p = ((uint64_t)t * NT + threadIdx.x) * NPOS;
    const bool inside = p < rs.total_bases;
    valid = inside ? window_valid_mask16(rs.starts32, p, rs.K, rs.total_bases) : 0u;
    if (NPOS < 16) valid &= (1u << NPOS) - 1u;
#pragma unroll
    for (int j = 0; j < NPOS / 2; j++) rk[j] = 0;
    Window16<W> win;
    if (NPOS == 16) load_window16<W>(rs.bases32, inside ? p : 0ull, rs.K, win);
    else load_window_at<W>(rs.bases32, inside ? p : 0ull, rs.K, win);
    extractN<W, NPOS>(win, rs.K, [&](int j, const Key<W>& c, bool) {
      key[j] = c;
      const uint32_t d = dg(c);
      if (FILTER) valid &= ~((uint32_t)((d - dg.flo) >= dg.fwidth) << j);
      const uint32_t r = atoms_add_if(cnt_a + 4 * d, 1u, valid & (1u << j));
      rk[j >> 1] |= r << ((j & 1) * 16);
      between(j);
    });
  };
  __syncthreads();
  extract_rank(t0, cnt2_a, [](int) {});
  for (uint32_t t = t0; t < t1; t++) {
    const uint32_t cur = (t - t0) & 1u;
    uint32_t* cnt = cnt2 + cur * bins;
    uint32_t* cnt_next = cnt2 + (cur ^ 1u) * bins;
    const uint32_t cnt_a = cnt2_a + cur * 4u * (uint32_t)bins, cnt_next_a = cnt2_a + (cur ^ 1u) * 4u * (uint32_t)bins;
    __syncthreads();
    const uint32_t tile_n = tile_scan<NT>(bins, G, Gabs, cnt, cnt_next, scratch);
    constexpr int PB = NPOS >= 8 ? 8 : NPOS;
#pragma unroll
    for (int j0 = 0; j0 < NPOS; j0 += PB) {
      uint32_t first[PB];
#pragma unroll
      for (int j = j0; j < j0 + PB; j++) first[j - j0] = lds_u32(cnt_a + 4 * dg(key[j]));
#pragma unroll
      for (int j = j0; j < j0 + PB; j++) {
        const uint32_t slot = first[j - j0] + ((rk[j >> 1] >> ((j & 1) * 16)) & 0xFFFFu);
        SmemElem<Key<W>>::st_if(stage_a + slot * ES, key[j], valid & (1u << j));
      }
    }
    __syncthreads();
    Key<W> kq[4];
    unsigned long long gq[4];
    auto write_out = [&](int j) {
      if ((j & 3) == 1) {
#pragma unroll
        for (int u = 0; u < 4; u++) kq[u] = lds_key<W>(stage_a + ((uint32_t)(j - 1 + u) * NT + threadIdx.x) * ES);
      } else if ((j & 3) == 2) {
#pragma unroll
        for (int u = 0; u < 4; u++) gq[u] = lds_u64(G_a + 8 * dg(kq[u]));
      } else if ((j & 3) == 3) {
#pragma unroll
        for (int u = 0; u < 4; u++) {
          const uint32_t i = (uint32_t)(j - 3 + u) * NT + threadIdx.x;
          stg_if(out + gq[u] + i, kq[u], (uint32_t)(i < tile_n), pol_st);
        }
      }
    };
    if (t + 1 < t1) {
      if (t + 2 < t1) {
        const uint64_t pn = ((uint64_t)(t + 2) * NT + threadIdx.x) * NPOS;
        if (pn < rs.total_bases) {
          if ((threadIdx.x % (128 / NPOS)) == 0) prefetch_l1(rs.bases32 + (pn >> 4));
          if ((threadIdx.x % (256 / NPOS)) == 0) prefetch_l1(rs.starts32 + (pn >> 5));
        }
      }
      extract_rank(t + 1, cnt_next_a, write_out);
    } else {
#pragma unroll
      for (int j = 0; j < NPOS; j++) write_out(j);
    }
  }
}

template <typename Out, typename In>
struct ElemCvt;
template <typename T>
struct ElemCvt<T, T> {
  __device__ __forceinline__ static T cvt(const T& e, int, int) { return e; }
};
template <>
struct ElemCvt<uint32_t, Key<1>> {
  __device__ __forceinline__ static uint32_t cvt(const Key<1>& e, int pad, int rem) {
    return (uint32_t)(e.w[0] << pad) & lowmask32(rem);
  }
};

template <typename Elem> struct TileItems { static constexpr int N = sizeof(Elem) <= 8 ? 16 : (sizeof(Elem) <= 16 ? 8 : 5); };

template <typename Elem, int NT, int MODE>
__global__ void __launch_bounds__(NT) k_hist_keys(const Elem* __restrict__ src, LevelPlan lp, DigitFn<MODE> dg,
                                                  uint32_t* __restrict__ chunksum, DigitFn<MODE> dgw = DigitFn<MODE>{}, int d2 = 0,
                                                  uint32_t* __restrict__ sub = nullptr) {
  extern __shared__ __align__(16) unsigned char smem_raw[];
  uint32_t* hist = (uint32_t*)smem_raw;
  const int bins = lp.bins;
  const int hbins = bins << d2;
  for (int i = threadIdx.x; i < hbins; i += NT) hist[i] = 0;
  __syncthreads();
  if (blockIdx.x >= lp.seg_chunk0[lp.n_segments]) return;
  int s; uint32_t t0, t1;
  chunk_tiles(lp, blockIdx.x, s, t0, t1);
  const uint64_t seg_lo = lp.seg_start[s], seg_hi = lp.seg_start[s + 1];
  const uint64_t e0 = seg_lo + (uint64_t)(t0 - lp.seg_tile0[s]) * lp.tile_elems;
  uint64_t e1 = seg_lo + (uint64_t)(t1 - lp.seg_tile0[s]) * lp.tile_elems;
  if (e1 > seg_hi) e1 = seg_hi;
  constexpr int U = 4;
  const uint32_t hist_a = smem_u32(hist);
  for (uint64_t base = e0; base < e1; base += (uint64_t)NT * U) {
    Elem r[U];
#pragma unroll
    for (int u = 0; u < U; u++) {
      const uint64_t i = base + (uint64_t)u * NT + threadIdx.x;
      if (i < e1) r[u] = src[i];
    }
#pragma unroll
    for (int u = 0; u < U; u++) {
      const uint64_t i = base + (uint64_t)u * NT + threadIdx.x;
      if (i < e1) reds_add(hist_a + 4 * (d2 ? dgw(r[u]) : dg(r[u])), 1u);
    }
  }
  __syncthreads();
  uint32_t* row = chunksum + (size_t)blockIdx.x * bins;
  if (d2 == 0) {
    for (int i = threadIdx.x; i < bins; i += NT) row[i] = hist[i];
  } else {
    uint32_t* gsub = sub + ((size_t)s * bins << d2);
    for (int i = threadIdx.x; i < bins; i += NT) {
      uint32_t t = 0;
      for (int j = 0; j < (1 << d2); j++) {
        const uint32_t v = hist[(i << d2) | j];
        if (v) atomicAdd(&gsub[(i << d2) | j], v);
        t += v;
      }
      row[i] = t;
    }
  }
}

template <typename ElemIn, typename ElemOut, int NT, int MODE, bool FILTER>
__global__ void __launch_bounds__(NT, (NT <= 512 ? 2 : 1)) k_scatter_keys(const ElemIn* __restrict__ src, LevelPlan lp, DigitFn<MODE> dg,
                                                     const uint32_t* __restrict__ chunkpref,
                                                     const uint64_t* __restrict__ bstart64, int out_pad, int out_rem,
                                                     ElemOut* __restrict__ out) {
  extern __shared__ __align__(16) unsigned char smem_raw[];
  ElemIn* stage; uint32_t* cnt2; unsigned long long* G; unsigned long long* Gabs; uint32_t* scratch;
  const int bins = lp.bins;
  scatter_smem_carve<ElemIn>(smem_raw, lp.tile_elems, bins, stage, cnt2, G, Gabs, scratch);
  if (blockIdx.x >= lp.seg_chunk0[lp.n_segments]) return;
  int s; uint32_t t0, t1;
  chunk_tiles(lp, blockIdx.x, s, t0, t1);
  const uint64_t seg_lo = lp.seg_start[s], seg_hi = lp.seg_start[s + 1];
  chunk_begin<NT>(chunkpref + (size_t)blockIdx.x * bins, bstart64, bstart64 ? 0ull : seg_lo, bins, Gabs, cnt2);
  constexpr int ITEMS = TileItems<ElemIn>::N;
  constexpr uint32_t ES = (uint32_t)sizeof(ElemIn);
  const uint32_t stage_a = smem_u32(stage), G_a = smem_u32(G), cnt2_a = smem_u32(cnt2);
  const uint64_t chunk_e0 = seg_lo + (uint64_t)(t0 - lp.seg_tile0[s]) * lp.tile_elems;
  const uint64_t pol_ld = APGK_LD_HINT ? l2_policy_evict_first() : 0ull;
  const uint64_t pol_st = APGK_ST_HINT == 1 ? l2_policy_evict_last() : (APGK_ST_HINT == 2 ? l2_policy_evict_first() : 0ull);
  ElemIn r[ITEMS];
  uint32_t rk[(ITEMS + 1) / 2];
  uint32_t live = 0;
  auto load_tile = [&](uint32_t t) {
    const uint64_t e0 = chunk_e0 + (uint64_t)(t - t0) * lp.tile_elems;
    live = 0;
#pragma unroll
    for (int u = 0; u < ITEMS; u++) {
      const uint64_t i = e0 + (uint64_t)u * NT + threadIdx.x;
      if (i < seg_hi) { r[u] = ldg_stream(src + i, pol_ld); live |= 1u << u; }
      else r[u] = ElemIn{};
    }
  };
  auto rank_tile = [&](uint32_t cnt_a) {
#pragma unroll
    for (int u = 0; u < (ITEMS + 1) / 2; u++) rk[u] = 0;
#pragma unroll
    for (int u = 0; u < ITEMS; u++) {
      const uint32_t d = dg(r[u]);
      if (FILTER) live &= ~((uint32_t)((d - dg.flo) >= dg.fwidth) << u);
      const uint32_t rr = atoms_add_if(cnt_a + 4 * d, 1u, live & (1u << u));
      rk[u >> 1] |= rr << ((u & 1) * 16);
    }
  };
  __syncthreads();
  load_tile(t0);
  rank_tile(cnt2_a);
  for (uint32_t t = t0; t < t1; t++) {
    const uint32_t cur = (t - t0) & 1u;
    uint32_t* cnt = cnt2 + cur * bins;
    uint32_t* cnt_next = cnt2 + (cur ^ 1u) * bins;
    const uint32_t cnt_a = cnt2_a + cur * 4u * (uint32_t)bins, cnt_next_a = cnt2_a + (cur ^ 1u) * 4u * (uint32_t)bins;
    __syncthreads();
    const uint32_t tile_n = tile_scan<NT>(bins, G, Gabs, cnt, cnt_next, scratch);
    {
      constexpr int PB = ITEMS >= 8 ? 8 : ITEMS;
#pragma unroll
      for (int u0 = 0; u0 < ITEMS; u0 += PB) {
        uint32_t first[PB];
#pragma unroll
        for (int u = u0; u < u0 + PB && u < ITEMS; u++) first[u - u0] = lds_u32(cnt_a + 4 * dg(r[u]));
#pragma unroll
        for (int u = u0; u < u0 + PB && u < ITEMS; u++) {
          const uint32_t slot = first[u - u0] + ((rk[u >> 1] >> ((u & 1) * 16)) & 0xFFFFu);
          SmemElem<ElemIn>::st_if(stage_a + slot * ES, r[u], live & (1u << u));
        }
      }
    }
    __syncthreads();
    const bool more = t + 1 < t1;
#if APGK_SK_EARLY
    if (more) load_tile(t + 1);
#else
    if (more) {
      const uint64_t i = chunk_e0 + (uint64_t)(t + 1 - t0) * lp.tile_elems + (uint64_t)threadIdx.x * (128 / ES);
      if (i < seg_hi && threadIdx.x * (128 / ES) < lp.tile_elems) prefetch_l2(src + i);
    }
#endif
    {
      constexpr int WB = ITEMS >= 4 ? 4 : ITEMS;
#pragma unroll
      for (int u0 = 0; u0 < ITEMS; u0 += WB) {
        ElemIn e[WB];
        unsigned long long g[WB];
#pragma unroll
        for (int u = u0; u < u0 + WB && u < ITEMS; u++) e[u - u0] = SmemElem<ElemIn>::ld(stage_a + ((uint32_t)u * NT + threadIdx.x) * ES);
#pragma unroll
        for (int u = u0; u < u0 + WB && u < ITEMS; u++) g[u - u0] = lds_u64(G_a + 8 * dg(e[u - u0]));
#pragma unroll
        for (int u = u0; u < u0 + WB && u < ITEMS; u++) {
          const uint32_t i = (uint32_t)u * NT + threadIdx.x;
          stg_if(out + g[u - u0] + i, ElemCvt<ElemOut, ElemIn>::cvt(e[u - u0], out_pad, out_rem), (uint32_t)(i < tile_n), pol_st);
        }
      }
    }
#if !APGK_SK_EARLY
    if (more) load_tile(t + 1);
#endif
    if (more) rank_tile(cnt_next_a);
  }
}

__device__ __forceinline__ void bulk_s2g(void* gdst, uint32_t ssrc, uint32_t bytes) {
  asm volatile("cp.async.bulk.global.shared::cta.bulk_group [%0], [%1], %2;" ::"l"(gdst), "r"(ssrc), "r"(bytes) : "memory");
}
__device__ __forceinline__ void bulk_commit() { asm volatile("cp.async.bulk.commit_group;" ::: "memory"); }
__device__ __forceinline__ void bulk_wait_read0() { asm volatile("cp.async.bulk.wait_group.read 0;" ::: "memory"); }
__device__ __forceinline__ void fence_async_smem() { asm volatile("fence.proxy.async.shared::cta;" ::: "memory"); }

template <typename Elem> struct BulkUnit {
  static constexpr uint32_t ES = (uint32_t)sizeof(Elem);
  static constexpr uint32_t U = ES % 16 == 0 ? 1u : (ES % 8 == 0 ? 2u : 4u);
};
template <typename ElemOut>
__host__ __device__ inline uint32_t scatter_bulk_stage_slots(uint32_t tile_elems, int bins) {
  return tile_elems + 2u * BulkUnit<ElemOut>::U * (uint32_t)bins;
}
template <typename ElemOut>
inline size_t scatter_bulk_smem_bytes(uint32_t tile_elems, int bins) {
  return (((size_t)scatter_bulk_stage_slots<ElemOut>(tile_elems, bins) * sizeof(ElemOut) + 15) & ~(size_t)15) + (size_t)bins * 24 + 40 * 4;
}

template <typename ElemIn, typename ElemOut, int NT, int MODE, bool FILTER>
__global__ void __launch_bounds__(NT, (NT <= 512 ? 2 : 1)) k_scatter_keys_bulk(const ElemIn* __restrict__ src, LevelPlan lp, DigitFn<MODE> dg,
                                                          const uint32_t* __restrict__ chunkpref,
                                                          const uint64_t* __restrict__ bstart64, int out_pad, int out_rem,
                                                          ElemOut* __restrict__ out) {
  extern __shared__ __align__(16) unsigned char smem_raw[];
  constexpr uint32_t ESO = (uint32_t)sizeof(ElemOut);
  constexpr uint32_t U = BulkUnit<ElemOut>::U;
  constexpr int NCAR = U > 1 ? (int)U - 1 : 1;
  const int bins = lp.bins;
  ElemOut* stage; uint32_t* cnt2; unsigned long long* G; unsigned long long* Gabs; uint32_t* scratch;
  scatter_smem_carve<ElemOut>(smem_raw, scatter_bulk_stage_slots<ElemOut>(lp.tile_elems, bins), bins, stage, cnt2, G, Gabs, scratch);
  if (blockIdx.x >= lp.seg_chunk0[lp.n_segments]) return;
  int s; uint32_t t0, t1;
  chunk_tiles(lp, blockIdx.x, s, t0, t1);
  const uint64_t seg_lo = lp.seg_start[s], seg_hi = lp.seg_start[s + 1];
  chunk_begin<NT>(chunkpref + (size_t)blockIdx.x * bins, bstart64, bstart64 ? 0ull : seg_lo, bins, Gabs, cnt2);
  constexpr int ITEMS = TileItems<ElemIn>::N;
  const uint32_t stage_a = smem_u32(stage), cnt2_a = smem_u32(cnt2);
  const uint64_t chunk_e0 = seg_lo + (uint64_t)(t0 - lp.seg_tile0[s]) * lp.tile_elems;
  const uint64_t pol_ld = APGK_LD_HINT ? l2_policy_evict_first() : 0ull;
  const bool owner = (int)threadIdx.x < bins;
  ElemIn r[ITEMS];
  uint32_t rk[(ITEMS + 1) / 2];
  uint32_t live = 0;
  auto load_tile = [&](uint32_t t) {
    const uint64_t e0 = chunk_e0 + (uint64_t)(t - t0) * lp.tile_elems;
    live = 0;
#pragma unroll
    for (int u = 0; u < ITEMS; u++) {
      const uint64_t i = e0 + (uint64_t)u * NT + threadIdx.x;
      if (i < seg_hi) { r[u] = ldg_stream(src + i, pol_ld); live |= 1u << u; }
      else r[u] = ElemIn{};
    }
  };
  auto rank_tile = [&](uint32_t cnt_a) {
#pragma unroll
    for (int u = 0; u < (ITEMS + 1) / 2; u++) rk[u] = 0;
#pragma unroll
    for (int u = 0; u < ITEMS; u++) {
      const uint32_t d = dg(r[u]);
      if (FILTER) live &= ~((uint32_t)((d - dg.flo) >= dg.fwidth) << u);
      const uint32_t rr = atoms_add_if(cnt_a + 4 * d, 1u, live & (1u << u));
      rk[u >> 1] |= rr << ((u & 1) * 16);
    }
  };
  __syncthreads();
  unsigned long long ga = owner ? Gabs[threadIdx.x] : 0ull;
  uint32_t hrem = owner ? (U - ((uint32_t)ga & (U - 1))) & (U - 1) : 0u;
  ElemOut car[NCAR];
#pragma unroll
  for (int i = 0; i < NCAR; i++) car[i] = ElemOut{};
  load_tile(t0);
  rank_tile(cnt2_a);
  for (uint32_t t = t0; t < t1; t++) {
    const uint32_t cur = (t - t0) & 1u;
    uint32_t* cnt = cnt2 + cur * bins;
    uint32_t* cnt_next = cnt2 + (cur ^ 1u) * bins;
    const uint32_t cnt_a = cnt2_a + cur * 4u * (uint32_t)bins, cnt_next_a = cnt2_a + (cur ^ 1u) * 4u * (uint32_t)bins;
    __syncthreads();
    const uint32_t c = owner ? cnt[threadIdx.x] : 0u;
    const uint32_t ph = (uint32_t)ga & (U - 1);
    uint32_t total;
    const uint32_t S = block_excl_scan1<NT>(c ? (ph + c + (U - 1)) & ~(U - 1) : 0u, scratch, total);
    if (owner) {
      cnt[threadIdx.x] = S + ph;
      cnt_next[threadIdx.x] = 0;
      if (c && hrem == 0) {
#pragma unroll
        for (int i = 0; i < NCAR; i++)
          if ((uint32_t)i < ph) SmemElem<ElemOut>::st(stage_a + (S + i) * ESO, car[i]);
      }
    }
    __syncthreads();
    {
      constexpr int PB = ITEMS >= 8 ? 8 : ITEMS;
#pragma unroll
      for (int u0 = 0; u0 < ITEMS; u0 += PB) {
        uint32_t first[PB];
#pragma unroll
        for (int u = u0; u < u0 + PB && u < ITEMS; u++) first[u - u0] = lds_u32(cnt_a + 4 * dg(r[u]));
#pragma unroll
        for (int u = u0; u < u0 + PB && u < ITEMS; u++) {
          const uint32_t slot = first[u - u0] + ((rk[u >> 1] >> ((u & 1) * 16)) & 0xFFFFu);
          SmemElem<ElemOut>::st_if(stage_a + slot * ESO, ElemCvt<ElemOut, ElemIn>::cvt(r[u], out_pad, out_rem), live & (1u << u));
        }
      }
    }
    fence_async_smem();
    __syncthreads();
    if (c) {
      uint32_t start, m;
      unsigned long long gidx;
      if (hrem) {
        const uint32_t x = hrem < c ? hrem : c;
        for (uint32_t i = 0; i < x; i++) out[ga + i] = SmemElem<ElemOut>::ld(stage_a + (S + ph + i) * ESO);
        hrem -= x;
        start = ph + x; gidx = ga + x; m = c - x;
      } else { start = 0; gidx = ga - ph; m = ph + c; }
      const uint32_t body = m & ~(U - 1);
      if (body) bulk_s2g(out + gidx, stage_a + (S + start) * ESO, body * ESO);
      if (hrem == 0) {
#pragma unroll
        for (int i = 0; i < NCAR; i++)
          if ((uint32_t)i < m - body) car[i] = SmemElem<ElemOut>::ld(stage_a + (S + start + body + i) * ESO);
      }
      ga += c;
    }
    bulk_commit();
    if (t + 1 < t1) {
      load_tile(t + 1);
      rank_tile(cnt_next_a);
    }
    bulk_wait_read0();
  }
  if (owner && hrem == 0) {
    const uint32_t kc = (uint32_t)ga & (U - 1);
#pragma unroll
    for (int i = 0; i < NCAR; i++)
      if ((uint32_t)i < kc) out[ga - kc + i] = car[i];
  }
}

template <int NT>
__device__ __forceinline__ unsigned long long block_excl_scan_u64(unsigned long long v, unsigned long long* scratch ) {
  const int lane = threadIdx.x & 31, wid = threadIdx.x >> 5;
  unsigned long long incl = v;
#pragma unroll
  for (int o = 1; o < 32; o <<= 1) {
    const unsigned long long u = __shfl_up_sync(0xffffffffu, incl, o);
    if (lane >= o) incl += u;
  }
  __syncthreads();
  if (lane == 31) scratch[wid] = incl;
  __syncthreads();
  if (wid == 0) {
    unsigned long long t = lane < NT / 32 ? scratch[lane] : 0ull, it = t;
#pragma unroll
    for (int o = 1; o < 32; o <<= 1) {
      const unsigned long long u = __shfl_up_sync(0xffffffffu, it, o);
      if (lane >= o) it += u;
    }
    scratch[lane] = it - t;
    if (lane == 31) scratch[32] = it;
  }
  __syncthreads();
  return incl - v + scratch[wid];
}

constexpr int PLAN_NT = 1024;
__global__ void __launch_bounds__(PLAN_NT) k_plan_range(const unsigned long long* __restrict__ tot, int n_seg, int s_lo, int s_hi,
                                                         uint32_t tile_elems, uint32_t chunk_tiles,
                                                         unsigned long long* __restrict__ seg_start, uint32_t* __restrict__ seg_tile0,
                                                         uint32_t* __restrict__ seg_chunk0, unsigned long long* __restrict__ info) {
  __shared__ unsigned long long scratch[34];
  __shared__ unsigned long long carry[4];
  if (threadIdx.x == 0) { carry[0] = carry[1] = carry[2] = carry[3] = 0; }
  __syncthreads();
  unsigned int bad = 0;
  for (int s0 = 0; s0 < n_seg; s0 += PLAN_NT) {
    const int s = s0 + (int)threadIdx.x;
    const unsigned long long all = s < n_seg ? tot[s] : 0ull;
    const unsigned long long n = (s >= s_lo && s < s_hi) ? all : 0ull;
    if (all >= (1ull << 32)) bad = 1;
    const unsigned long long tiles = (n + tile_elems - 1) / tile_elems;
    const unsigned long long chunks = (tiles + chunk_tiles - 1) / chunk_tiles;
    const unsigned long long e_n = block_excl_scan_u64<PLAN_NT>(n, scratch);
    const unsigned long long t_n = scratch[32];
    const unsigned long long e_t = block_excl_scan_u64<PLAN_NT>(tiles, scratch);
    const unsigned long long t_t = scratch[32];
    const unsigned long long e_c = block_excl_scan_u64<PLAN_NT>(chunks, scratch);
    const unsigned long long t_c = scratch[32];
    const unsigned long long e_a = block_excl_scan_u64<PLAN_NT>(all, scratch);
    const unsigned long long t_a = scratch[32];
    (void)e_a;
    if (s < n_seg) {
      seg_start[s] = carry[0] + e_n;
      if (seg_tile0) seg_tile0[s] = (uint32_t)(carry[1] + e_t);
      if (seg_chunk0) seg_chunk0[s] = (uint32_t)(carry[2] + e_c);
    }
    __syncthreads();
    if (threadIdx.x == 0) { carry[0] += t_n; carry[1] += t_t; carry[2] += t_c; carry[3] += t_a; }
    __syncthreads();
  }
  if (threadIdx.x == 0) {
    seg_start[n_seg] = carry[0];
    if (seg_tile0) seg_tile0[n_seg] = (uint32_t)carry[1];
    if (seg_chunk0) seg_chunk0[n_seg] = (uint32_t)carry[2];
    if (info) { info[0] = carry[0]; info[1] = carry[3]; }
  }
  if (bad && info) atomicOr(&info[2], 1ull);
}

template <int NT>
__global__ void __launch_bounds__(NT) k_segscan(LevelPlan lp, uint32_t* __restrict__ chunksum,
                                                unsigned long long* __restrict__ segtot64,
                                                uint32_t* __restrict__ bstart32,
                                                unsigned long long* __restrict__ bofs , int fold) {
  __shared__ uint32_t scratch[34];
  __shared__ unsigned long long carry_s;
  const int s = blockIdx.x;
  const int bins = lp.bins;
  const uint32_t c0 = lp.seg_chunk0[s], c1 = lp.seg_chunk0[s + 1];
  if (threadIdx.x == 0) carry_s = 0;
  __syncthreads();
  for (int d0 = 0; d0 < bins; d0 += NT) {
    const int d = d0 + threadIdx.x;
    unsigned long long run = 0;
    if (d < bins) {
      for (uint32_t c = c0; c < c1; c++) run += chunksum[(size_t)c * bins + d];
      segtot64[(size_t)s * bins + d] = run;
    }
    uint32_t excl = block_excl_scan<NT>((uint32_t)run, scratch);
    unsigned long long carry = carry_s;
    if (d < bins) {
      const uint32_t bs = (uint32_t)(carry + excl);
      bstart32[(size_t)s * bins + d] = bs;
      if (bofs) bofs[(size_t)s * bins + d] = lp.seg_start[s] + carry + excl;
      uint32_t pre = fold ? bs : 0u;
      for (uint32_t c = c0; c < c1; c++) {
        const uint32_t v = chunksum[(size_t)c * bins + d];
        chunksum[(size_t)c * bins + d] = pre;
        pre += v;
      }
    }
    __syncthreads();
    if (threadIdx.x == 0) carry_s = carry + scratch[32];
    __syncthreads();
  }
}

}
```

include/apgk.h:

```cpp
#ifndef APGK_H
#define APGK_H
#include <stddef.h>
#include <stdint.h>

#ifdef __cplusplus
extern "C" {
#endif

#define APGK_OK 0
#define APGK_E_ARG (-1)
#define APGK_E_CUDA (-2)
#define APGK_E_NOMEM (-3)
#define APGK_E_STATE (-4)
#define APGK_E_RANGE (-5)

#define APGK_WANT_SPECTRUM 1u
#define APGK_WANT_COUNTS 2u
#define APGK_ASYNC_INGEST 4u

#define APGK_MAX_K 96

typedef struct apgk_ctx apgk_ctx;

typedef struct {
  int32_t K;
  int32_t device;
  uint32_t flags;
  int32_t prefix_bits;
  uint64_t reserve_bases;
  uint64_t max_round_keys;
  uint64_t max_inner_keys;
} apgk_config;

typedef struct {
  uint64_t genome_len;
  uint64_t seed_g, seed_p, seed_q, seed_r, seed_e;
  uint32_t read_len;
  uint32_t err_per_200;
} apgk_synth_params;

int apgk_create(const apgk_config* cfg, apgk_ctx** out);
void apgk_destroy(apgk_ctx* ctx);
const char* apgk_last_error(const apgk_ctx* ctx);
int apgk_words_per_kmer(int K);

int apgk_reset(apgk_ctx* ctx);

int apgk_add_reads(apgk_ctx* ctx, const uint8_t* packed, const uint64_t* off, uint64_t n_reads);
int apgk_add_reads_uniform(apgk_ctx* ctx, const uint8_t* packed, uint64_t first_base, uint64_t n_reads,
                           uint32_t read_len);
int apgk_synth_reads(apgk_ctx* ctx, const apgk_synth_params* p, uint64_t r0, uint64_t n_reads);
int apgk_export_reads(apgk_ctx* ctx, uint8_t* packed_out);
int apgk_read_store_info(const apgk_ctx* ctx, uint64_t* total_bases, uint64_t* n_reads);

int apgk_finish(apgk_ctx* ctx);

int apgk_totals(const apgk_ctx* ctx, uint64_t* n_instances, uint64_t* n_distinct);
int apgk_spectrum(apgk_ctx* ctx, const uint64_t** spec, uint64_t* len);
int apgk_spectrum_sparse(apgk_ctx* ctx, const uint64_t** freq, const uint64_t** n_kmers, uint64_t* n);
int apgk_counts_device(apgk_ctx* ctx, const uint64_t** d_kmers, const uint32_t** d_counts, uint64_t* n_distinct);
int apgk_counts_copy(apgk_ctx* ctx, uint64_t first, uint64_t n, uint64_t* kmers_out, uint32_t* counts_out);

int apgk_release_temp(apgk_ctx* ctx);
int apgk_reserve_table(apgk_ctx* ctx, uint64_t n_records);
int apgk_prefix_range(apgk_ctx* ctx, int32_t prefix_bits, uint64_t prefix, uint64_t* first, uint64_t* n);

int apgk_lookup(apgk_ctx* ctx, const uint64_t* kmers, uint64_t n, int canonicalise, uint32_t* counts_out);
int apgk_read_freqs(apgk_ctx* ctx, uint64_t first_base, uint64_t n_bases, uint32_t* out);
int apgk_read_freqs_device(apgk_ctx* ctx, uint32_t* d_out, float* ms3);

int apgk_build_occurrences(apgk_ctx* ctx);
int apgk_occurrences_info(const apgk_ctx* ctx, uint64_t* n_occ, uint64_t* n_big_runs, float* ms5);
int apgk_occurrences_device(apgk_ctx* ctx, const uint64_t** d_run_off, const uint64_t** d_occ, uint64_t* n_occ);
int apgk_occurrences_copy(apgk_ctx* ctx, uint64_t first_kmer, uint64_t n_kmers, uint64_t* run_off_out,
                          uint32_t* read_id_out, int32_t* pos_out);

int apgk_owner_plan(apgk_ctx* ctx, uint32_t n_ranks, uint64_t* counts_out);
int apgk_owner_scatter(apgk_ctx* ctx, uint64_t* d_keys_out);
int apgk_key_buffer(apgk_ctx* ctx, uint64_t n_keys, uint64_t** d_ptr);
int apgk_owner_of(int K, const uint64_t* kmers, uint64_t n, uint32_t n_ranks, uint32_t* owner_out);
int apgk_finish_keys_device(apgk_ctx* ctx, const uint64_t* d_keys, uint64_t n);
int apgk_spectrum_device(apgk_ctx* ctx, uint64_t** d_spec, uint64_t* len);
int apgk_spectrum_reload(apgk_ctx* ctx);

int apgk_window_upper(const apgk_ctx* ctx, uint64_t* upper);
int apgk_choose_prefix_bits(apgk_ctx* ctx, uint64_t upper, int32_t* prefix_bits);
int apgk_partition(apgk_ctx* ctx, int32_t prefix_bits);
int apgk_partition_range(apgk_ctx* ctx, int32_t prefix_bits, int32_t d0_lo, int32_t d0_hi);
int apgk_level0_totals(apgk_ctx* ctx, uint64_t* totals_out, uint32_t cap, uint32_t* n_level0, uint64_t* round_capacity);
int apgk_partition_info(apgk_ctx* ctx, const uint64_t** d_bucket_sizes, uint64_t* n_buckets, void** d_elems,
                        uint32_t* elem_bytes, uint64_t* n_elems);
int apgk_count_pieces(apgk_ctx* ctx, const void* d_recv, uint32_t n_src, const uint32_t* d_sizes_all,
                      const uint64_t* seg_off, uint64_t bucket_lo, uint64_t bucket_hi, int32_t split_bits);

int apgk_count_pieces_peer(apgk_ctx* ctx, const void* const* d_src_base, uint32_t n_src, const uint32_t* d_sizes_all,
                           const uint64_t* src_off, uint64_t bucket_lo, uint64_t bucket_hi, int32_t split_bits,
                           const uint32_t* d_sub_sizes);
int apgk_partition_subsizes(apgk_ctx* ctx, int32_t split_bits, int32_t* effective_bits, const uint32_t** d_sub_sizes);
int apgk_partition_export(apgk_ctx* ctx, uint8_t handle_out[64]);
int apgk_peer_open(apgk_ctx* ctx, const uint8_t handle[64], void** d_ptr);
int apgk_peer_close(apgk_ctx* ctx, void* d_ptr);

typedef struct apgk_group apgk_group;
#define APGK_GROUP_ID_BYTES 128
int apgk_group_unique_id(uint8_t id_out[APGK_GROUP_ID_BYTES]);
int apgk_group_join(apgk_ctx* ctx, const uint8_t id[APGK_GROUP_ID_BYTES], int32_t rank, int32_t world, apgk_group** out);
int apgk_group_local(apgk_ctx* const* ctxs, int32_t n, apgk_group** out);
void apgk_group_destroy(apgk_group* g);
const char* apgk_group_last_error(const apgk_group* g);
int apgk_group_count(apgk_group* g);
int apgk_group_totals(const apgk_group* g, uint64_t* n_instances, uint64_t* n_distinct);
int apgk_group_spectrum_sparse(apgk_group* g, const uint64_t** freq, const uint64_t** n_kmers, uint64_t* n);
typedef struct {
  int32_t world, n_rounds, n_outer_rounds, prefix_bits, split_bits, peer_exchange;
  uint64_t shard_instances;
  uint64_t remote_bytes;
  float gather_ms;
  float step_ms;
} apgk_group_stats;
int apgk_group_stats_get(const apgk_group* g, apgk_group_stats* out);
typedef struct {
  int32_t n_batches;
  uint64_t n_queries;
  uint64_t remote_bytes;
  float sweep_ms, exchange_ms, scatter_ms, total_ms;
} apgk_group_freq_stats;
int apgk_group_read_freqs_device(apgk_group* g, uint32_t* const* d_out, const uint64_t* first_base,
                                 const uint64_t* n_bases, apgk_group_freq_stats* stats);

#define APGK_N_STAGES 14
int apgk_stage_ms(const apgk_ctx* ctx, float* ms_out );
const char* apgk_stage_name(int i);
uint64_t apgk_kernel_launches(const apgk_ctx* ctx);
void apgk_reset_counters(apgk_ctx* ctx);
int apgk_geometry(const apgk_ctx* ctx, int32_t* out8);
int apgk_device_alloc(apgk_ctx* ctx, void** p, size_t bytes);
int apgk_device_free(apgk_ctx* ctx, void* p);
int apgk_device_copy_to_host(apgk_ctx* ctx, void* dst_host, const void* src_dev, size_t bytes);
int apgk_host_alloc(void** p, size_t bytes);
int apgk_host_free(void* p);

int apgk_debug_counters(apgk_ctx* ctx, uint64_t* out8, int reset);
int apgk_debug_host_extract(const uint8_t* packed, const uint64_t* off, uint64_t n_reads, int K,
                            uint64_t* kmers_out , uint8_t* valid_out );
int apgk_debug_host_canonical(int K, const uint64_t* kmers, uint64_t n, uint64_t* out);
int apgk_debug_host_topdigits(const uint8_t* packed, const uint64_t* off, uint64_t n_reads, int K, int D,
                              uint32_t* digits_out );
int apgk_debug_host_table_find(int K, const uint64_t* sorted_kmers, uint64_t n, int prefix_bits, const uint64_t* queries,
                               uint64_t n_q, uint64_t* idx_out);
int apgk_debug_host_synth(const apgk_synth_params* p, uint64_t r0, uint64_t n_reads, uint8_t* packed_out);
int apgk_debug_host_splitters(const uint32_t* bucket_sizes, uint32_t n_buckets, uint32_t world, uint32_t bucket_cost,
                              uint32_t* bounds_out);

#ifdef __cplusplus
}
#endif
#endif
```

Before: 53.14.

## Replace window validity loop with bit-smear and specialize digit extraction mode

Rewrites window_valid_mask16 to compute the invalid-window mask with funnel shifts and log-step OR smearing instead of iterating over read-start bits, templated on max K. Adds a DIGIT_BITS_LSH mode so the common W=1 digit path skips the extra shift when kind is zero, dispatched at launch time. Simplifies scatter tile load bounds and position arithmetic, and adds host debug entry points to check the new mask against the old loop. This increases template instantiations, and the bit tricks risk subtle correctness errors at edge positions.

New measurement: 50.45 (median of 6 runs). 0.949x the previous value.

```diff
diff --git a/allpathslg_b200/_lib.py b/allpathslg_b200/_lib.py
--- a/allpathslg_b200/_lib.py
+++ b/allpathslg_b200/_lib.py
@@ -110,6 +110,8 @@
     "apgk_debug_host_table_find": (C.c_int, [C.c_int, _vp, C.c_uint64, C.c_int, _vp, C.c_uint64, _vp]),
     "apgk_debug_host_splitters": (C.c_int, [_vp, C.c_uint32, C.c_uint32, C.c_uint32, _vp]),
     "apgk_debug_host_synth": (C.c_int, [C.POINTER(SynthParams), C.c_uint64, C.c_uint64, _vp]),
+    "apgk_debug_host_valid_mask": (C.c_int, [_vp, C.c_uint64, C.c_int, _vp, C.c_uint64, _vp, _vp]),
+    "apgk_debug_host_digit": (C.c_int, [C.c_int, C.c_int, C.c_int, C.c_int, _vp, C.c_uint64, _vp]),
 }
 
 _lib = None
diff --git a/allpathslg_b200/csrc/apgk.cu b/allpathslg_b200/csrc/apgk.cu
--- a/allpathslg_b200/csrc/apgk.cu
+++ b/allpathslg_b200/csrc/apgk.cu
@@ -440,9 +440,9 @@
   return APGK_OK;
 }
 
-template <typename ElemB, int W>
+template <typename ElemB, int W, int MODE>
 struct ScatterSel {
-  static auto kernel() { return k_scatter_keys<Key<W>, ElemB, Geo<W>::NT1, DIGIT_BITS, false>; }
+  static auto kernel() { return k_scatter_keys<Key<W>, ElemB, Geo<W>::NT1, MODE, false>; }
 };
 
 __global__ void k_accumulate_u64(unsigned long long* __restrict__ dst, const unsigned long long* __restrict__ src, uint64_t n) {
@@ -510,13 +510,22 @@
   CU(c->chunksum0.ensure((size_t)hp0.lp.n_chunks * bins0 * 4));
   stage_begin(c, ST_HIST0);
   if (dev_keys) {
-    k_hist_keys<Key<W>, Geo<W>::NT1, DIGIT_BITS><<<hp0.lp.n_chunks, Geo<W>::NT1, bins0 * 4, c->stream>>>(
-        dev_keys, hp0.lp, dg0, c->chunksum0.as<uint32_t>());
+    with_digit_mode<W>([&](auto m) {
+      constexpr int M = decltype(m)::value;
+      k_hist_keys<Key<W>, Geo<W>::NT1, M><<<hp0.lp.n_chunks, Geo<W>::NT1, bins0 * 4, c->stream>>>(
+          dev_keys, hp0.lp, dg0.template with_mode<M>(), c->chunksum0.as<uint32_t>());
+    }, dg0);
   } else {
     const int top_bits = (g.pad == 0 && g.D0 <= 16 && c->cfg.K >= (g.D0 + 1) / 2 && !getenv("APGK_NO_TOPDIGITS")) ? g.D0 : 0;
+    auto hist_reads = [&](uint32_t n_chunks, uint32_t chunk0) {
+      with_digit_mode<W>([&](auto m) {
+        constexpr int M = decltype(m)::value;
+        k_hist_reads<W, Geo<W>::NT0, M><<<n_chunks, Geo<W>::NT0, bins0 * 4, c->stream>>>(
+            read_store(c), dg0.template with_mode<M>(), hp0.lp, top_bits, c->chunksum0.as<uint32_t>(), chunk0);
+      }, dg0);
+    };
     if (c->n_slices == 0) {
-      k_hist_reads<W, Geo<W>::NT0, DIGIT_BITS><<<hp0.lp.n_chunks, Geo<W>::NT0, bins0 * 4, c->stream>>>(
-          read_store(c), dg0, hp0.lp, top_bits, c->chunksum0.as<uint32_t>());
+      hist_reads(hp0.lp.n_chunks, 0);
     } else {
       const uint64_t reach = (uint64_t)c->cfg.K + 256;
       uint32_t c_lo = 0;
@@ -528,8 +537,7 @@
           c_hi = (uint32_t)std::min<uint64_t>(hp0.lp.n_chunks, safe / ((uint64_t)tile0 * hp0.lp.chunk_tiles));
         }
         if (c_hi > c_lo) {
-          k_hist_reads<W, Geo<W>::NT0, DIGIT_BITS><<<c_hi - c_lo, Geo<W>::NT0, bins0 * 4, c->stream>>>(
-              read_store(c), dg0, hp0.lp, top_bits, c->chunksum0.as<uint32_t>(), c_lo);
+          hist_reads(c_hi - c_lo, c_lo);
           c->launches++;
           c_lo = c_hi;
         }
@@ -566,27 +574,29 @@
   dg0.flo = (uint32_t)lo; dg0.fwidth = (uint32_t)(hi - lo);
   stage_begin(c, ST_SCATTER0);
   const size_t sm = scatter_smem_bytes<Key<W>>(tile0, bins0);
-  if (dev_keys) {
-    auto launch = [&](auto kern) -> int {
-      { int rc = kernel_setup(c, kern, Geo<W>::NT1, sm, nullptr); if (rc) return rc; }
-      kern<<<hp0.lp.n_chunks, Geo<W>::NT1, sm, c->stream>>>(dev_keys, hp0.lp, dg0, c->chunksum0.as<uint32_t>(),
-                                                            c->bstart64.as<uint64_t>(), 0, 0, c->A.as<Key<W>>());
-      return APGK_OK;
-    };
-    int rc = filter ? launch(k_scatter_keys<Key<W>, Key<W>, Geo<W>::NT1, DIGIT_BITS, true>)
-                    : launch(k_scatter_keys<Key<W>, Key<W>, Geo<W>::NT1, DIGIT_BITS, false>);
-    if (rc) return rc;
-  } else {
+  int rc = with_digit_mode<W>([&](auto m) -> int {
+    constexpr int M = decltype(m)::value;
+    const DigitFn<M> dg = dg0.template with_mode<M>();
+    if (dev_keys) {
+      auto launch = [&](auto kern) -> int {
+        { int rc = kernel_setup(c, kern, Geo<W>::NT1, sm, nullptr); if (rc) return rc; }
+        kern<<<hp0.lp.n_chunks, Geo<W>::NT1, sm, c->stream>>>(dev_keys, hp0.lp, dg, c->chunksum0.as<uint32_t>(),
+                                                              c->bstart64.as<uint64_t>(), 0, 0, c->A.as<Key<W>>());
+        return APGK_OK;
+      };
+      return filter ? launch(k_scatter_keys<Key<W>, Key<W>, Geo<W>::NT1, M, true>)
+                    : launch(k_scatter_keys<Key<W>, Key<W>, Geo<W>::NT1, M, false>);
+    }
     auto launch = [&](auto kern) -> int {
       { int rc = kernel_setup(c, kern, Geo<W>::NTS, sm, nullptr); if (rc) return rc; }
-      kern<<<hp0.lp.n_chunks, Geo<W>::NTS, sm, c->stream>>>(read_store(c), dg0, hp0.lp, c->chunksum0.as<uint32_t>(),
+      kern<<<hp0.lp.n_chunks, Geo<W>::NTS, sm, c->stream>>>(read_store(c), dg, hp0.lp, c->chunksum0.as<uint32_t>(),
                                                             c->bstart64.as<uint64_t>(), c->A.as<Key<W>>());
       return APGK_OK;
     };
-    int rc = filter ? launch(k_scatter_reads<W, Geo<W>::NTS, DIGIT_BITS, true, Geo<W>::NPOS>)
-                    : launch(k_scatter_reads<W, Geo<W>::NTS, DIGIT_BITS, false, Geo<W>::NPOS>);
-    if (rc) return rc;
-  }
+    return filter ? launch(k_scatter_reads<W, Geo<W>::NTS, M, true, Geo<W>::NPOS>)
+                  : launch(k_scatter_reads<W, Geo<W>::NTS, M, false, Geo<W>::NPOS>);
+  }, dg0);
+  if (rc) return rc;
   LAUNCHED();
   stage_end(c, ST_SCATTER0);
   return APGK_OK;
@@ -629,11 +639,16 @@
   }
   stage_begin(c, ST_HIST1);
   {
-    auto kern = k_hist_keys<Key<W>, Geo<W>::NT1, DIGIT_BITS>;
-    const size_t smh = ((size_t)bins1 << d2) * 4;
-    { int rc = kernel_setup(c, kern, Geo<W>::NT1, smh, nullptr); if (rc) return rc; }
-    kern<<<chunks_bound, Geo<W>::NT1, smh, c->stream>>>(a_src, lp, dg1, c->chunksum.as<uint32_t>(), dgw, d2,
-                                                        d2 > 0 ? c->sub_sizes.as<uint32_t>() : nullptr);
+    int rc = with_digit_mode<W>([&](auto m) -> int {
+      constexpr int M = decltype(m)::value;
+      auto kern = k_hist_keys<Key<W>, Geo<W>::NT1, M>;
+      const size_t smh = ((size_t)bins1 << d2) * 4;
+      { int rc = kernel_setup(c, kern, Geo<W>::NT1, smh, nullptr); if (rc) return rc; }
+      kern<<<chunks_bound, Geo<W>::NT1, smh, c->stream>>>(a_src, lp, dg1.template with_mode<M>(), c->chunksum.as<uint32_t>(),
+                                                          dgw.template with_mode<M>(), d2, d2 > 0 ? c->sub_sizes.as<uint32_t>() : nullptr);
+      return APGK_OK;
+    }, dg1, dgw);
+    if (rc) return rc;
     LAUNCHED();
   }
   stage_end(c, ST_HIST1);
@@ -648,18 +663,23 @@
     const char* eb = getenv("APGK_BULK");
     const bool bulk = eb && !strcmp(eb, "1");
     const size_t smb = scatter_bulk_smem_bytes<ElemB>(tile, bins1);
-    if (bulk && sizeof(ElemB) == 4 && smb <= 200 * 1024 && bins1 <= Geo<W>::NT1) {
-      auto kern = k_scatter_keys_bulk<Key<W>, ElemB, Geo<W>::NT1, DIGIT_BITS, false>;
-      { int rc = kernel_setup(c, kern, Geo<W>::NT1, smb, nullptr); if (rc) return rc; }
-      kern<<<chunks_bound, Geo<W>::NT1, smb, c->stream>>>(a_src, lp, dg1, c->chunksum.as<uint32_t>(), nullptr, g.pad, g.REM,
-                                                          c->B.as<ElemB>());
-    } else {
-      auto kern = ScatterSel<ElemB, W>::kernel();
-      const size_t sm = scatter_smem_bytes<Key<W>>(tile, bins1);
-      { int rc = kernel_setup(c, kern, Geo<W>::NT1, sm, nullptr); if (rc) return rc; }
-      kern<<<chunks_bound, Geo<W>::NT1, sm, c->stream>>>(a_src, lp, dg1, c->chunksum.as<uint32_t>(), nullptr, g.pad, g.REM,
-                                                         c->B.as<ElemB>());
-    }
+    int rc = with_digit_mode<W>([&](auto m) -> int {
+      constexpr int M = decltype(m)::value;
+      if (bulk && sizeof(ElemB) == 4 && smb <= 200 * 1024 && bins1 <= Geo<W>::NT1) {
+        auto kern = k_scatter_keys_bulk<Key<W>, ElemB, Geo<W>::NT1, M, false>;
+        { int rc = kernel_setup(c, kern, Geo<W>::NT1, smb, nullptr); if (rc) return rc; }
+        kern<<<chunks_bound, Geo<W>::NT1, smb, c->stream>>>(a_src, lp, dg1.template with_mode<M>(), c->chunksum.as<uint32_t>(),
+                                                            nullptr, g.pad, g.REM, c->B.as<ElemB>());
+      } else {
+        auto kern = ScatterSel<ElemB, W, M>::kernel();
+        const size_t sm = scatter_smem_bytes<Key<W>>(tile, bins1);
+        { int rc = kernel_setup(c, kern, Geo<W>::NT1, sm, nullptr); if (rc) return rc; }
+        kern<<<chunks_bound, Geo<W>::NT1, sm, c->stream>>>(a_src, lp, dg1.template with_mode<M>(), c->chunksum.as<uint32_t>(),
+                                                           nullptr, g.pad, g.REM, c->B.as<ElemB>());
+      }
+      return APGK_OK;
+    }, dg1);
+    if (rc) return rc;
     LAUNCHED();
   }
   stage_end(c, ST_SCATTER1);
@@ -2349,6 +2369,57 @@
   return APGK_OK;
 }
 
+namespace {
+uint32_t valid_mask16_loop(const uint32_t* starts32, uint64_t p, int K, uint64_t total_bases) {
+  if (p + (uint64_t)K > total_bases) return 0u;
+  uint32_t ok = 0xFFFFu;
+  const uint64_t room = total_bases - (uint64_t)K - p;
+  if (room < 15) ok = (2u << (uint32_t)room) - 1u;
+  if (K < 2) return ok;
+  const uint64_t lo = p + 1, hi = p + (uint64_t)K + 14;
+  uint32_t inv = 0;
+  for (uint64_t wi = lo >> 5; wi <= (hi >> 5); wi++) {
+    uint32_t bits = starts32[wi];
+    if (wi == (lo >> 5)) bits &= 0xFFFFFFFFu << (uint32_t)(lo & 31);
+    if (wi == (hi >> 5)) bits &= 0xFFFFFFFFu >> (31u - (uint32_t)(hi & 31));
+    while (bits) {
+      const int b = __builtin_ctz(bits);
+      bits &= bits - 1;
+      const int st = (int)((wi << 5) + (uint64_t)b - p);
+      const int j0 = st - K + 1 > 0 ? st - K + 1 : 0;
+      const int j1 = st - 1 < 15 ? st - 1 : 15;
+      if (j0 <= j1) inv |= ((2u << j1) - 1u) & ~((1u << j0) - 1u);
+    }
+  }
+  return ok & ~inv;
+}
+}
+
+int apgk_debug_host_valid_mask(const uint32_t* starts32, uint64_t total_bases, int K, const uint64_t* p, uint64_t n,
+                               uint32_t* out, uint32_t* ref_out) {
+  if (!starts32 || !p || !out || !ref_out || K < 1 || K > APGK_MAX_K) return APGK_E_ARG;
+  const uint64_t nw = (total_bases + 31) / 32;
+  std::vector<uint32_t> st(nw + 16, 0);
+  std::copy(starts32, starts32 + nw, st.begin());
+  for (uint64_t i = 0; i < n; i++) {
+    if (p[i] >= total_bases) return APGK_E_ARG;
+    out[i] = window_valid_mask16(st.data(), p[i], K, total_bases);
+    ref_out[i] = valid_mask16_loop(st.data(), p[i], K, total_bases);
+  }
+  return APGK_OK;
+}
+
+int apgk_debug_host_digit(int K, int pos, int len, int pad, const uint64_t* keys, uint64_t n, uint32_t* out) {
+  if (!keys || !out || K < 1 || K > 32 || len < 1 || len > 32 || pos < 0 || pad < 0 || pos + len > 2 * K + pad || pad > 64 - 2 * K)
+    return APGK_E_ARG;
+  const DigitFn<DIGIT_BITS> dg = make_digit_fn<DIGIT_BITS>(DigitSpec{DIGIT_BITS, pos, len, pad, 0});
+  with_digit_mode<1>([&](auto m) {
+    const DigitFn<decltype(m)::value> f = dg.template with_mode<decltype(m)::value>();
+    for (uint64_t i = 0; i < n; i++) out[i] = f(Key<1>{{keys[i]}});
+  }, dg);
+  return APGK_OK;
+}
+
 int apgk_debug_host_canonical(int K, const uint64_t* kmers, uint64_t n, uint64_t* out) {
   if (K < 1 || K > APGK_MAX_K) return APGK_E_ARG;
   const int W = words_for(K);
diff --git a/allpathslg_b200/csrc/extract.cuh b/allpathslg_b200/csrc/extract.cuh
--- a/allpathslg_b200/csrc/extract.cuh
+++ b/allpathslg_b200/csrc/extract.cuh
@@ -109,30 +109,36 @@
   }
 }
 
+template <int KMAX = 96>
 APGK_HD uint32_t window_valid_mask16(const uint32_t* __restrict__ starts32, uint64_t p, int K, uint64_t total_bases) {
   if (p + (uint64_t)K > total_bases) return 0u;
   uint32_t ok = 0xFFFFu;
   const uint64_t room = total_bases - (uint64_t)K - p;
   if (room < 15) ok = (2u << (uint32_t)room) - 1u;
   if (K < 2) return ok;
-  const uint64_t lo = p + 1, hi = p + (uint64_t)K + 14;
-  uint32_t inv = 0;
-  for (uint64_t wi = lo >> 5; wi <= (hi >> 5); wi++) {
-    uint32_t bits = starts32[wi];
-    if (wi == (lo >> 5)) bits &= 0xFFFFFFFFu << (uint32_t)(lo & 31);
-    if (wi == (hi >> 5)) bits &= 0xFFFFFFFFu >> (31u - (uint32_t)(hi & 31));
-    while (bits) {
-#ifdef __CUDA_ARCH__
-      const int b = __ffs((int)bits) - 1;
-#else
-      const int b = __builtin_ctz(bits);
-#endif
-      bits &= bits - 1;
-      const int s = (int)((wi << 5) + (uint64_t)b - p);
-      const int j0 = s - K + 1 > 0 ? s - K + 1 : 0;
-      const int j1 = s - 1 < 15 ? s - 1 : 15;
-      if (j0 <= j1) inv |= ((2u << j1) - 1u) & ~((1u << j0) - 1u);
+  const uint32_t w = (uint32_t)K - 1u;
+  const uint32_t* s = starts32 + ((p + 1) >> 5);
+  const uint32_t sh = (uint32_t)(p + 1) & 31u;
+  const uint32_t x0 = funnel_r(s[0], s[1], sh), x1 = funnel_r(s[1], s[2], sh);
+  uint32_t inv;
+  if (KMAX <= 50 || w <= 49) {
+    uint64_t r = (uint64_t)x0 | ((uint64_t)x1 << 32);
+    uint32_t span = 1;
+#pragma unroll
+    for (int e = 0; e < 5; e++) {
+      if ((2u << e) <= w) { r |= r >> (1u << e); span = 2u << e; }
     }
+    inv = (uint32_t)r | funnel_r((uint32_t)r, (uint32_t)(r >> 32), w - span);
+  } else {
+    uint32_t a = x0 & 0x7FFFu;
+    a |= a >> 1; a |= a >> 2; a |= a >> 4; a |= a >> 8;
+    const uint32_t x2 = funnel_r(s[2], s[3], sh);
+    const uint32_t mid = (x0 >> 15) | (x1 & lowmask32((int)(w < 64 ? w : 64u) - 32)) | (w > 64 ? x2 & lowmask32((int)w - 64) : 0u);
+    const uint64_t q = p + (uint64_t)K;
+    const uint32_t* sy = starts32 + (q >> 5);
+    uint32_t y = funnel_r(sy[0], sy[1], (uint32_t)q & 31u) & 0x7FFFu;
+    y |= y << 1; y |= y << 2; y |= y << 4; y |= y << 8;
+    inv = a | (y << 1) | (mid ? 0xFFFFu : 0u);
   }
   return ok & ~inv;
 }
diff --git a/allpathslg_b200/csrc/partition.cuh b/allpathslg_b200/csrc/partition.cuh
--- a/allpathslg_b200/csrc/partition.cuh
+++ b/allpathslg_b200/csrc/partition.cuh
@@ -1,6 +1,7 @@
 #pragma once
 #include "extract.cuh"
 #include <cstdio>
+#include <type_traits>
 
 #ifdef APGK_CHECKS
 #define APGK_CHECK(cond, ...) do { if (!(cond)) { printf(__VA_ARGS__); } } while (0)
@@ -149,6 +150,7 @@
 
 constexpr int DIGIT_BITS = 0;
 constexpr int DIGIT_OWNER = 1;
+constexpr int DIGIT_BITS_LSH = 2;
 
 struct DigitSpec {
   int mode;
@@ -166,14 +168,19 @@
   uint32_t n_ranks;
   uint32_t flo, fwidth;
   template <int W>
-  __device__ __forceinline__ uint32_t operator()(const Key<W>& k) const {
+  APGK_HD uint32_t operator()(const Key<W>& k) const {
     if constexpr (MODE == DIGIT_OWNER) return key_owner(k, n_ranks);
     else if constexpr (W == 1) {
       const uint32_t t = (uint32_t)(k.w[0] >> (sh & 63));
-      return (t << (kind & 31)) & mask;
+      if constexpr (MODE == DIGIT_BITS_LSH) return (t << (kind & 31)) & mask;
+      else return t & mask;
     } else return key_bits(k, pos, len);
   }
-  __device__ __forceinline__ uint32_t operator()(uint32_t e) const { return (e >> rsh) & mask; }
+  APGK_HD uint32_t operator()(uint32_t e) const { return (e >> rsh) & mask; }
+  template <int M2>
+  DigitFn<M2> with_mode() const {
+    return DigitFn<M2>{kind, sh, mask, rsh, pos, len, n_ranks, flo, fwidth};
+  }
 };
 template <int MODE>
 inline DigitFn<MODE> make_digit_fn(const DigitSpec& ds) {
@@ -187,6 +194,13 @@
   f.flo = 0; f.fwidth = 0xFFFFFFFFu;
   return f;
 }
+template <int W, typename F, typename... D>
+inline auto with_digit_mode(F&& f, const D&... dgs) {
+  if constexpr (W == 1) {
+    if (((dgs.kind != 0) || ...)) return f(std::integral_constant<int, DIGIT_BITS_LSH>{});
+  }
+  return f(std::integral_constant<int, DIGIT_BITS>{});
+}
 
 template <int NT>
 __device__ __forceinline__ uint32_t block_excl_scan(uint32_t v, uint32_t* warp_scratch) {
@@ -285,12 +299,13 @@
   const uint32_t chunk = blockIdx.x + chunk0;
   chunk_tiles(lp, chunk, s, t0, t1);
   const uint32_t hist_a = smem_u32(hist);
+  const uint32_t tp = threadIdx.x * POS_PER_THREAD;
   for (uint32_t t = t0; t < t1; t++) {
-    const uint64_t p = ((uint64_t)t * NT + threadIdx.x) * POS_PER_THREAD;
+    const uint64_t p = (uint64_t)t * (NT * POS_PER_THREAD) + tp;
     if (p < rs.total_bases) {
-      const uint32_t valid = window_valid_mask16(rs.starts32, p, rs.K, rs.total_bases);
+      const uint32_t valid = window_valid_mask16<32 * W>(rs.starts32, p, rs.K, rs.total_bases);
       if (valid) {
-        if (MODE == DIGIT_BITS && top_bits > 0) {
+        if (MODE != DIGIT_OWNER && top_bits > 0) {
           top_digits16(rs.bases32, p, rs.K, top_bits, [&](int j, uint32_t d) {
             if ((valid >> j) & 1u) reds_add(hist_a + 4 * d, 1u);
           });
@@ -388,10 +403,11 @@
   Key<W> key[NPOS];
   uint32_t rk[NPOS / 2];
   uint32_t valid = 0;
+  const uint32_t tp = threadIdx.x * NPOS;
   auto extract_rank = [&](uint32_t t, uint32_t cnt_a, auto&& between) {
-    const uint64_t p = ((uint64_t)t * NT + threadIdx.x) * NPOS;
+    const uint64_t p = (uint64_t)t * (NT * NPOS) + tp;
     const bool inside = p < rs.total_bases;
-    valid = inside ? window_valid_mask16(rs.starts32, p, rs.K, rs.total_bases) : 0u;
+    valid = inside ? window_valid_mask16<32 * W>(rs.starts32, p, rs.K, rs.total_bases) : 0u;
     if (NPOS < 16) valid &= (1u << NPOS) - 1u;
 #pragma unroll
     for (int j = 0; j < NPOS / 2; j++) rk[j] = 0;
@@ -448,7 +464,7 @@
     };
     if (t + 1 < t1) {
       if (t + 2 < t1) {
-        const uint64_t pn = ((uint64_t)(t + 2) * NT + threadIdx.x) * NPOS;
+        const uint64_t pn = (uint64_t)(t + 2) * (NT * NPOS) + tp;
         if (pn < rs.total_bases) {
           if ((threadIdx.x % (128 / NPOS)) == 0) prefetch_l1(rs.bases32 + (pn >> 4));
           if ((threadIdx.x % (256 / NPOS)) == 0) prefetch_l1(rs.starts32 + (pn >> 5));
@@ -466,12 +482,12 @@
 struct ElemCvt;
 template <typename T>
 struct ElemCvt<T, T> {
-  __device__ __forceinline__ static T cvt(const T& e, int, int) { return e; }
+  __device__ __forceinline__ static T cvt(const T& e, int, uint32_t) { return e; }
 };
 template <>
 struct ElemCvt<uint32_t, Key<1>> {
-  __device__ __forceinline__ static uint32_t cvt(const Key<1>& e, int pad, int rem) {
-    return (uint32_t)(e.w[0] << pad) & lowmask32(rem);
+  __device__ __forceinline__ static uint32_t cvt(const Key<1>& e, int pad, uint32_t mask) {
+    return (uint32_t)(e.w[0] << pad) & mask;
   }
 };
 
@@ -496,6 +512,7 @@
   if (e1 > seg_hi) e1 = seg_hi;
   constexpr int U = 4;
   const uint32_t hist_a = smem_u32(hist);
+#pragma unroll 1
   for (uint64_t base = e0; base < e1; base += (uint64_t)NT * U) {
     Elem r[U];
 #pragma unroll
@@ -546,17 +563,21 @@
   const uint32_t stage_a = smem_u32(stage), G_a = smem_u32(G), cnt2_a = smem_u32(cnt2);
   const uint64_t chunk_e0 = seg_lo + (uint64_t)(t0 - lp.seg_tile0[s]) * lp.tile_elems;
   const uint64_t pol_ld = APGK_LD_HINT ? l2_policy_evict_first() : 0ull;
+  const int cvt_pad = MODE == DIGIT_BITS_LSH ? out_pad : 0;
+  const uint32_t cvt_mask = lowmask32(out_rem);
   const uint64_t pol_st = APGK_ST_HINT == 1 ? l2_policy_evict_last() : (APGK_ST_HINT == 2 ? l2_policy_evict_first() : 0ull);
   ElemIn r[ITEMS];
   uint32_t rk[(ITEMS + 1) / 2];
   uint32_t live = 0;
   auto load_tile = [&](uint32_t t) {
     const uint64_t e0 = chunk_e0 + (uint64_t)(t - t0) * lp.tile_elems;
+    const uint64_t left = seg_hi > e0 ? seg_hi - e0 : 0ull;
+    const uint32_t n = left < lp.tile_elems ? (uint32_t)left : lp.tile_elems;
+    const ElemIn* __restrict__ ts = src + e0 + threadIdx.x;
     live = 0;
 #pragma unroll
     for (int u = 0; u < ITEMS; u++) {
-      const uint64_t i = e0 + (uint64_t)u * NT + threadIdx.x;
-      if (i < seg_hi) { r[u] = ldg_stream(src + i, pol_ld); live |= 1u << u; }
+      if (u * NT + threadIdx.x < n) { r[u] = ldg_stream(ts + u * NT, pol_ld); live |= 1u << u; }
       else r[u] = ElemIn{};
     }
   };
@@ -618,7 +639,7 @@
 #pragma unroll
         for (int u = u0; u < u0 + WB && u < ITEMS; u++) {
           const uint32_t i = (uint32_t)u * NT + threadIdx.x;
-          stg_if(out + g[u - u0] + i, ElemCvt<ElemOut, ElemIn>::cvt(e[u - u0], out_pad, out_rem), (uint32_t)(i < tile_n), pol_st);
+          stg_if(out + g[u - u0] + i, ElemCvt<ElemOut, ElemIn>::cvt(e[u - u0], cvt_pad, cvt_mask), (uint32_t)(i < tile_n), pol_st);
         }
       }
     }
@@ -670,17 +691,21 @@
   const uint32_t stage_a = smem_u32(stage), cnt2_a = smem_u32(cnt2);
   const uint64_t chunk_e0 = seg_lo + (uint64_t)(t0 - lp.seg_tile0[s]) * lp.tile_elems;
   const uint64_t pol_ld = APGK_LD_HINT ? l2_policy_evict_first() : 0ull;
+  const int cvt_pad = MODE == DIGIT_BITS_LSH ? out_pad : 0;
+  const uint32_t cvt_mask = lowmask32(out_rem);
   const bool owner = (int)threadIdx.x < bins;
   ElemIn r[ITEMS];
   uint32_t rk[(ITEMS + 1) / 2];
   uint32_t live = 0;
   auto load_tile = [&](uint32_t t) {
     const uint64_t e0 = chunk_e0 + (uint64_t)(t - t0) * lp.tile_elems;
+    const uint64_t left = seg_hi > e0 ? seg_hi - e0 : 0ull;
+    const uint32_t n = left < lp.tile_elems ? (uint32_t)left : lp.tile_elems;
+    const ElemIn* __restrict__ ts = src + e0 + threadIdx.x;
     live = 0;
 #pragma unroll
     for (int u = 0; u < ITEMS; u++) {
-      const uint64_t i = e0 + (uint64_t)u * NT + threadIdx.x;
-      if (i < seg_hi) { r[u] = ldg_stream(src + i, pol_ld); live |= 1u << u; }
+      if (u * NT + threadIdx.x < n) { r[u] = ldg_stream(ts + u * NT, pol_ld); live |= 1u << u; }
       else r[u] = ElemIn{};
     }
   };
@@ -733,7 +758,7 @@
 #pragma unroll
         for (int u = u0; u < u0 + PB && u < ITEMS; u++) {
           const uint32_t slot = first[u - u0] + ((rk[u >> 1] >> ((u & 1) * 16)) & 0xFFFFu);
-          SmemElem<ElemOut>::st_if(stage_a + slot * ESO, ElemCvt<ElemOut, ElemIn>::cvt(r[u], out_pad, out_rem), live & (1u << u));
+          SmemElem<ElemOut>::st_if(stage_a + slot * ESO, ElemCvt<ElemOut, ElemIn>::cvt(r[u], cvt_pad, cvt_mask), live & (1u << u));
         }
       }
     }
diff --git a/include/apgk.h b/include/apgk.h
--- a/include/apgk.h
+++ b/include/apgk.h
@@ -149,6 +149,9 @@
 int apgk_debug_host_table_find(int K, const uint64_t* sorted_kmers, uint64_t n, int prefix_bits, const uint64_t* queries,
                                uint64_t n_q, uint64_t* idx_out);
 int apgk_debug_host_synth(const apgk_synth_params* p, uint64_t r0, uint64_t n_reads, uint8_t* packed_out);
+int apgk_debug_host_valid_mask(const uint32_t* starts32, uint64_t total_bases, int K, const uint64_t* p, uint64_t n,
+                               uint32_t* out, uint32_t* ref_out);
+int apgk_debug_host_digit(int K, int pos, int len, int pad, const uint64_t* keys, uint64_t n, uint32_t* out);
 int apgk_debug_host_splitters(const uint32_t* bucket_sizes, uint32_t n_buckets, uint32_t world, uint32_t bucket_cost,
                               uint32_t* bounds_out);
 
```
